# al-mcintyre/mCaller

Measured on NVIDIA B200. Metric: per-read site calls/sec, higher is better.
Workload: dtype f64

## Files before the change

### include/mcaller_b200.h

```cpp
#ifndef MCALLER_B200_H
#define MCALLER_B200_H

#include <stdint.h>

#ifdef __cplusplus
extern "C" {
#endif

#define MC_ABI_VERSION 3

#define MC_TILE_BYTES 3840
#define MC_TEXT_PAD 4096
#define MC_MAXK 8

enum {
    MC_OK = 0,
    MC_EINVAL = -1,
    MC_ECUDA = -2,
    MC_ECAPACITY = -3
};

typedef struct mc_refindex {
    int32_t n_contigs;
    int32_t k;
    const uint8_t *d_names;
    const int32_t *d_name_off;
    const int64_t *d_base;
    const int32_t *d_len;
    const uint32_t *d_site_fwd;
    const uint32_t *d_site_rev;
    const uint32_t *d_cand;
    const uint32_t *d_rank_fwd;
    const uint32_t *d_rank_rev;
    const uint8_t *d_bases;
    int64_t total_bits;
} mc_refindex;

typedef struct mc_record {
    uint32_t line_lo;
    uint16_t line_hi;
    uint16_t name_off;
    int32_t pos;
    int32_t event_idx;
    double diff;
    uint16_t name_len;
    uint16_t contig;
    uint8_t flags;
    uint8_t kbits_fwd;
    uint8_t kbits_rev;
    uint8_t pad;
} mc_record;

#define MC_RF_EQ 1u
#define MC_RF_CAND 2u
#define MC_RF_BADNUM 4u
#define MC_RF_BADIDX 8u
#define MC_RF_RAW 16u
#define MC_RF_NEWREAD 32u
#define MC_RF_SEGKNOWN 64u

enum {
    MC_C_LINES = 0,
    MC_C_KEPT,
    MC_C_RECORDS,
    MC_C_SHORT,
    MC_C_UNKNOWN_CONTIG,
    MC_C_NNN,
    MC_C_BADPOS,
    MC_C_LONGLINE,
    MC_C_OVERFLOW,
    MC_C_RUN_CURSOR,
    MC_C_QUIET,
    MC_C_COUNT = 16
};

typedef struct mc_call {
    int64_t read_off;
    double prob;
    double feat[MC_MAXK + 1];
    int32_t read_len;
    int32_t mpos;
    int32_t site;
    uint32_t close_rec;
    uint16_t win_contig;
    uint16_t chrom_contig;
    uint8_t kind;
    uint8_t rev;
    uint8_t n_empty;
    uint8_t empty_mask;
    uint8_t model_sel;
    uint8_t label;
    uint8_t err;
    uint8_t pad0;
    uint32_t seg;
    uint32_t pad1;
    uint32_t pad2;
} mc_call;

enum { MC_CALL = 0, MC_TOO_MANY_SKIPS = 1, MC_MULTI_M = 2, MC_NONE = 3  };
#define MC_CE_CONTEXT 1u
#define MC_CE_MODELKEY 2u
#define MC_CE_BADNUM 4u
#define MC_CE_COLUMN 8u
#define MC_CE_SPACING 16u

enum { MC_MLP = 0, MC_LR = 1, MC_GNB = 2, MC_RF = 3 };
enum { MC_ACT_IDENTITY = 0, MC_ACT_LOGISTIC = 1, MC_ACT_TANH = 2, MC_ACT_RELU = 3 };
typedef struct mc_model {
    int32_t kind;
    int32_t n_in;
    int32_t n_layers;
    int32_t hidden_act;
    int32_t sizes[8];
    const double *d_weights;
    const double *d_biases;
    int32_t n_trees;
    int32_t max_nodes;
    const int32_t *d_tree_off;
    const int32_t *d_left;
    const int32_t *d_right;
    const int32_t *d_feature;
    const double *d_threshold;
    const double *d_leaf_p1;
} mc_model;

typedef struct mc_qual_entry {
    uint64_t hash;
    uint32_t check;
    uint32_t len;
    double qual;
} mc_qual_entry;


int mc_version(void);
int mc_sizeof(int what);
const char *mc_last_error(void);

int mc_read_u64(const uint64_t *d_src, int64_t n, uint64_t *h_dst, void *stream);

int mc_scan(const uint8_t *d_text, int64_t nbytes, const mc_refindex *ref, int dense,
            mc_record *d_rec, int64_t rec_cap, uint32_t *d_tile_tab , uint32_t *d_run_tab ,
            uint64_t *d_counters, void *stream);

int mc_scan_run_len(int64_t nbytes);

int mc_scan_set_run_len(int run_len);

int64_t mc_num_tiles(int64_t nbytes);

int64_t mc_workspace_bytes(int64_t n);

int mc_order_records(const uint8_t *d_text, int64_t nbytes, const mc_refindex *ref, const uint32_t *d_tile_tab, int64_t n_tiles,
                     uint32_t *d_run_tab, int run_len, const mc_record *d_rec_in, int64_t rec_in_cap, const uint64_t *d_scan_counters,
                     mc_record *d_rec_out, int64_t rec_out_cap, uint64_t *d_n_out, uint32_t *d_seg_flags ,
                     uint32_t *d_run_first , void *d_ws, void *stream);

int mc_segment_reads(const uint8_t *d_text, mc_record *d_rec, const uint64_t *d_n_records, int64_t rec_cap,
                     uint32_t *d_seg_flags , const uint32_t *d_run_first, int64_t n_runs,
                     uint32_t *d_seg_start, uint64_t *d_nseg, void *d_ws, void *stream);

int mc_segment_quality(const uint8_t *d_text, const mc_record *d_rec, const uint32_t *d_seg_start, const uint64_t *d_nseg,
                       int64_t seg_cap, const mc_qual_entry *d_table, int64_t table_size, double *d_seg_qual, uint64_t *d_err,
                       void *stream);

int mc_build_windows(const mc_record *d_rec, const uint64_t *d_n_records, int64_t rec_cap, const uint32_t *d_seg_start,
                     const uint64_t *d_nseg, int64_t seg_cap, const double *d_seg_qual, const mc_refindex *ref, int skip_thresh,
                     double qual_thresh, int two_models, mc_call *d_calls, int64_t call_cap, uint32_t *d_seg_count,
                     uint64_t *d_ncalls, void *d_ws, double *d_spill, int64_t spill_cap, void *stream);

typedef struct mc_carry {
    mc_call row;
    uint32_t valid;
    int32_t first_kept_contig;
    uint64_t chunks;
    uint64_t pad[6];
} mc_carry;
int mc_carry_reset(mc_carry *d_carry, void *stream);
int mc_carry_rows(mc_call *d_rows, const uint64_t *d_ncalls, const mc_record *d_rec, const uint64_t *d_n_records,
                  const uint32_t *d_seg_start, const uint64_t *d_nseg, const double *d_seg_qual, double qual_thresh,
                  mc_carry *d_carry, uint64_t *d_nrows_out, const uint64_t *d_abort, void *stream);
int mc_chunk_guard(const uint64_t *d_counters, int64_t rec_cap, const uint64_t *d_n_records, int64_t rec_out_cap,
                   const uint64_t *d_nseg, int64_t seg_cap, const uint64_t *d_ncalls, int64_t call_cap, uint64_t *d_abort,
                   uint64_t *d_sticky , void *stream);
int mc_carry_close(mc_carry *d_carry, int closing_contig, const int64_t *d_next_contigs, int from, int count, mc_call *d_row_out,
                   uint32_t *d_depth, uint32_t *d_meth, uint64_t *d_first, int64_t n_sites, uint64_t *d_row_base, void *stream);

int64_t mc_classify_workspace_bytes(int64_t row_cap);
int mc_classify(mc_call *d_calls, const uint64_t *d_nrows, int64_t row_cap, const mc_model *models, void *d_ws, void *stream);

int mc_hist_accumulate(const mc_call *d_calls, const uint64_t *d_nrows, int64_t row_cap, uint32_t *d_depth, uint32_t *d_meth,
                       uint64_t *d_first, int64_t n_sites, uint64_t *d_row_base, mc_call *d_odd, int64_t odd_cap, uint64_t *d_n_odd,
                       const uint64_t *d_abort , void *stream);

int mc_bed_select(const uint32_t *d_depth, const uint32_t *d_meth, int64_t n_sites, int64_t depth_thresh, double mod_thresh,
                  int control, uint8_t *d_flags, uint64_t *d_count, void *stream);

int mc_count_calls(const mc_call *d_calls, const uint64_t *d_nrows, int64_t row_cap, uint64_t *d_out, void *stream);

typedef struct mc_locus_entry {
    unsigned long long hash;
    unsigned long long first_off;
    unsigned long long check;
    uint32_t depth;
    uint32_t meth;
} mc_locus_entry;

typedef struct mc_diffs_row {
    uint64_t line_off;
    uint32_t slot;
    uint32_t values_off;
    uint32_t values_len;
    uint32_t prob_off;
    uint32_t prob_len;
    uint32_t pad;
} mc_diffs_row;
int mc_diffs_aggregate_ex(const uint8_t *d_text, int64_t nbytes, int64_t base_off, const uint64_t *d_posset, int64_t posset_size,
                          mc_locus_entry *d_table, int64_t table_size, uint64_t *d_counters, void *stream);
int mc_diffs_rehash(const mc_locus_entry *d_old, int64_t old_size, mc_locus_entry *d_table, int64_t table_size,
                    uint64_t *d_counters, void *stream);
int mc_diffs_rows(const uint8_t *d_text, int64_t nbytes, const uint64_t *d_posset, int64_t posset_size,
                  const mc_locus_entry *d_table, int64_t table_size, mc_diffs_row *d_rows, int64_t row_cap, uint64_t *d_nrows,
                  void *stream);
int mc_diffs_colstats(const uint8_t *d_text, const mc_diffs_row *d_rows, const uint32_t *d_order, int64_t n_rows,
                      const uint32_t *d_locus_off, int64_t n_loci, int ncols, double *d_vals, uint32_t *d_ncol,
                      double *d_stats, uint64_t *d_counters, void *stream);

int64_t mc_format_rows(const mc_call *h_calls, int64_t n_calls, const uint8_t *h_text, const uint8_t *carry_name,
                       int32_t carry_name_len, const char *const *contig_names, const char *const *marked_fwd,
                       const char *const *marked_rev, const int64_t *contig_len, int32_t n_contigs, int32_t k,
                       const char *base_label, const char *mod_label, int32_t with_prob, int32_t max_threads, char *out,
                       int64_t out_cap);

int64_t mc_fastq_tiles(int64_t nbytes);
int mc_fastq_index(const uint8_t *d_text, int64_t nbytes, uint32_t *d_tile_cnt, uint32_t *d_tile_off, uint64_t *d_line_start,
                   int64_t line_cap, uint64_t *d_n_newlines, void *d_ws, void *stream);
int mc_fastq_quality(const uint8_t *d_text, int64_t nbytes, const uint64_t *d_line_start, int64_t n_lines, mc_qual_entry *d_table,
                     int64_t table_size, uint32_t *d_owner, double *d_rec_mean, uint64_t *d_stats, void *stream);

#define MC_TRAIN_HIDDEN 100
#define MC_TRAIN_BATCH 200
typedef struct mc_train_job {
    const double *d_x;
    const double *d_y;
    double *d_w;
    double *d_loss_curve;
    int64_t idx_off;
    int32_t n, d;
    int32_t max_iter, n_iter_no_change;
    double alpha, lr, tol;
    double best_loss;
    int32_t n_iter, no_improve, stopped, pad;
} mc_train_job;

int mc_mlp_train_init(mc_train_job *d_jobs, int32_t n_jobs, void *stream);
int mc_mlp_train_epochs(mc_train_job *d_jobs, int32_t n_jobs, const int32_t *d_idx, int32_t epochs, void *stream);

typedef struct mc_synth_spec {
    uint64_t seed;
    int32_t n_contigs;
    int32_t len_min, len_max, p_skip, p_nnn, margin;
    int32_t meth;
    const uint8_t *d_names;
    const int32_t *d_name_off;
    const int32_t *d_contig_len;
    const int64_t *d_read_bounds;
    const int64_t *d_gbase;
    const uint8_t *d_genome;
    const uint32_t *d_meth_fwd;
    const uint32_t *d_meth_rev;
    const int32_t *d_model_mean;
    const int32_t *d_model_sd;
} mc_synth_spec;

int mc_synth_genome(const mc_synth_spec *spec, uint8_t *d_genome_out, int64_t total_bits, void *stream);
int mc_synth_sizes(const mc_synth_spec *spec, int64_t read0, int64_t n, int64_t n_total_reads, uint64_t *d_sizes, void *stream);
int mc_synth_write(const mc_synth_spec *spec, int64_t read0, int64_t n, int64_t n_total_reads, const uint64_t *d_offsets,
                   uint8_t *d_text, void *stream);

#ifdef __cplusplus
}
#endif
#endif
```

### mcaller_b200/_lib.py

```python
import ctypes as C
import os

import numpy as np

HERE = os.path.dirname(os.path.abspath(__file__))
LIB_PATH = os.environ.get("MCALLER_B200_LIB") or os.path.join(HERE, "libmcaller_b200.so")

MC_TILE_BYTES = 3840
MC_TEXT_PAD = 4096
MC_MAXK = 8
MC_C_COUNT = 16
COUNTER_NAMES = ["lines", "kept", "records", "short", "unknown_contig", "nnn", "badpos", "longline", "overflow", "run_cursor", "quiet_chunks"]

MC_ABI_VERSION = 3
MC_CALL, MC_TOO_MANY_SKIPS, MC_MULTI_M, MC_NONE = 0, 1, 2, 3
MC_CE_CONTEXT, MC_CE_MODELKEY, MC_CE_BADNUM, MC_CE_COLUMN, MC_CE_SPACING = 1, 2, 4, 8, 16
MC_MLP, MC_LR, MC_GNB, MC_RF = 0, 1, 2, 3
PENDING = 0xFFFFFFFF


class RefIndex(C.Structure):
    _fields_ = [("n_contigs", C.c_int32), ("k", C.c_int32), ("d_names", C.c_void_p), ("d_name_off", C.c_void_p),
                ("d_base", C.c_void_p), ("d_len", C.c_void_p), ("d_site_fwd", C.c_void_p), ("d_site_rev", C.c_void_p),
                ("d_cand", C.c_void_p), ("d_rank_fwd", C.c_void_p), ("d_rank_rev", C.c_void_p), ("d_bases", C.c_void_p),
                ("total_bits", C.c_int64)]


class Model(C.Structure):
    _fields_ = [("kind", C.c_int32), ("n_in", C.c_int32), ("n_layers", C.c_int32), ("hidden_act", C.c_int32),
                ("sizes", C.c_int32 * 8), ("d_weights", C.c_void_p), ("d_biases", C.c_void_p), ("n_trees", C.c_int32),
                ("max_nodes", C.c_int32), ("d_tree_off", C.c_void_p), ("d_left", C.c_void_p), ("d_right", C.c_void_p),
                ("d_feature", C.c_void_p), ("d_threshold", C.c_void_p), ("d_leaf_p1", C.c_void_p)]


class SynthSpec(C.Structure):
    _fields_ = [("seed", C.c_uint64), ("n_contigs", C.c_int32), ("len_min", C.c_int32), ("len_max", C.c_int32),
                ("p_skip", C.c_int32), ("p_nnn", C.c_int32), ("margin", C.c_int32), ("meth", C.c_int32),
                ("d_names", C.c_void_p), ("d_name_off", C.c_void_p), ("d_contig_len", C.c_void_p),
                ("d_read_bounds", C.c_void_p), ("d_gbase", C.c_void_p), ("d_genome", C.c_void_p),
                ("d_meth_fwd", C.c_void_p), ("d_meth_rev", C.c_void_p), ("d_model_mean", C.c_void_p),
                ("d_model_sd", C.c_void_p)]


RECORD_DTYPE = np.dtype([("line_lo", "<u4"), ("line_hi", "<u2"), ("name_off", "<u2"), ("pos", "<i4"), ("event_idx", "<i4"),
                         ("diff", "<f8"), ("name_len", "<u2"), ("contig", "<u2"), ("flags", "u1"), ("kbits_fwd", "u1"), ("kbits_rev", "u1"), ("pad", "u1")])
assert RECORD_DTYPE.itemsize == 32

CALL_DTYPE = np.dtype([("read_off", "<i8"), ("prob", "<f8"), ("feat", "<f8", (MC_MAXK + 1,)), ("read_len", "<i4"),
                       ("mpos", "<i4"), ("site", "<i4"), ("close_rec", "<u4"), ("win_contig", "<u2"), ("chrom_contig", "<u2"),
                       ("kind", "u1"), ("rev", "u1"), ("n_empty", "u1"), ("empty_mask", "u1"), ("model_sel", "u1"),
                       ("label", "u1"), ("err", "u1"), ("pad0", "u1"), ("seg", "<u4"), ("pad1", "<u4"), ("pad2", "<u4")])
assert CALL_DTYPE.itemsize == 128

class LocusEntry(C.Structure):
    _fields_ = [("hash", C.c_uint64), ("first_off", C.c_uint64), ("check", C.c_uint64), ("depth", C.c_uint32), ("meth", C.c_uint32)]


class TrainJob(C.Structure):
    _fields_ = [("d_x", C.c_void_p), ("d_y", C.c_void_p), ("d_w", C.c_void_p), ("d_loss_curve", C.c_void_p), ("idx_off", C.c_int64),
                ("n", C.c_int32), ("d", C.c_int32), ("max_iter", C.c_int32), ("n_iter_no_change", C.c_int32), ("alpha", C.c_double),
                ("lr", C.c_double), ("tol", C.c_double), ("best_loss", C.c_double), ("n_iter", C.c_int32), ("no_improve", C.c_int32),
                ("stopped", C.c_int32), ("pad", C.c_int32)]


MC_TRAIN_HIDDEN, MC_TRAIN_BATCH = 100, 200

CARRY_BYTES = 192

QUAL_DTYPE = np.dtype([("hash", "<u8"), ("check", "<u4"), ("len", "<u4"), ("qual", "<f8")])
assert QUAL_DTYPE.itemsize == 24
DIFFS_ROW_DTYPE = np.dtype([("line_off", "<u8"), ("slot", "<u4"), ("values_off", "<u4"), ("values_len", "<u4"), ("prob_off", "<u4"),
                            ("prob_len", "<u4"), ("pad", "<u4")])
assert DIFFS_ROW_DTYPE.itemsize == 32


class McallerCudaError(RuntimeError):
    pass


_lib = None

_PROTOS = {
    "mc_version": (C.c_int, []),
    "mc_sizeof": (C.c_int, [C.c_int]),
    "mc_last_error": (C.c_char_p, []),
    "mc_read_u64": (C.c_int, [C.c_void_p, C.c_int64, C.c_void_p, C.c_void_p]),
    "mc_scan": (C.c_int, [C.c_void_p, C.c_int64, C.POINTER(RefIndex), C.c_int, C.c_void_p, C.c_int64, C.c_void_p, C.c_void_p, C.c_void_p,
                          C.c_void_p]),
    "mc_scan_run_len": (C.c_int, [C.c_int64]),
    "mc_scan_set_run_len": (C.c_int, [C.c_int]),
    "mc_num_tiles": (C.c_int64, [C.c_int64]),
    "mc_workspace_bytes": (C.c_int64, [C.c_int64]),
    "mc_order_records": (C.c_int, [C.c_void_p, C.c_int64, C.POINTER(RefIndex), C.c_void_p, C.c_int64, C.c_void_p, C.c_int, C.c_void_p,
                                   C.c_int64, C.c_void_p, C.c_void_p, C.c_int64, C.c_void_p, C.c_void_p, C.c_void_p, C.c_void_p, C.c_void_p]),
    "mc_segment_reads": (C.c_int, [C.c_void_p, C.c_void_p, C.c_void_p, C.c_int64, C.c_void_p, C.c_void_p, C.c_int64, C.c_void_p, C.c_void_p,
                                   C.c_void_p, C.c_void_p]),
    "mc_segment_quality": (C.c_int, [C.c_void_p, C.c_void_p, C.c_void_p, C.c_void_p, C.c_int64, C.c_void_p, C.c_int64, C.c_void_p,
                                     C.c_void_p, C.c_void_p]),
    "mc_build_windows": (C.c_int, [C.c_void_p, C.c_void_p, C.c_int64, C.c_void_p, C.c_void_p, C.c_int64, C.c_void_p, C.POINTER(RefIndex),
                                   C.c_int, C.c_double, C.c_int, C.c_void_p, C.c_int64, C.c_void_p, C.c_void_p, C.c_void_p, C.c_void_p,
                                   C.c_int64, C.c_void_p]),
    "mc_carry_reset": (C.c_int, [C.c_void_p, C.c_void_p]),
    "mc_carry_rows": (C.c_int, [C.c_void_p, C.c_void_p, C.c_void_p, C.c_void_p, C.c_void_p, C.c_void_p, C.c_void_p, C.c_double, C.c_void_p,
                                C.c_void_p, C.c_void_p, C.c_void_p]),
    "mc_chunk_guard": (C.c_int, [C.c_void_p, C.c_int64, C.c_void_p, C.c_int64, C.c_void_p, C.c_int64, C.c_void_p, C.c_int64, C.c_void_p,
                                 C.c_void_p, C.c_void_p]),
    "mc_carry_close": (C.c_int, [C.c_void_p, C.c_int, C.c_void_p, C.c_int, C.c_int, C.c_void_p, C.c_void_p, C.c_void_p, C.c_void_p,
                                 C.c_int64, C.c_void_p, C.c_void_p]),
    "mc_classify_workspace_bytes": (C.c_int64, [C.c_int64]),
    "mc_classify": (C.c_int, [C.c_void_p, C.c_void_p, C.c_int64, C.POINTER(Model), C.c_void_p, C.c_void_p]),
    "mc_hist_accumulate": (C.c_int, [C.c_void_p, C.c_void_p, C.c_int64, C.c_void_p, C.c_void_p, C.c_void_p, C.c_int64, C.c_void_p,
                                     C.c_void_p, C.c_int64, C.c_void_p, C.c_void_p, C.c_void_p]),
    "mc_count_calls": (C.c_int, [C.c_void_p, C.c_void_p, C.c_int64, C.c_void_p, C.c_void_p]),
    "mc_bed_select": (C.c_int, [C.c_void_p, C.c_void_p, C.c_int64, C.c_int64, C.c_double, C.c_int, C.c_void_p, C.c_void_p, C.c_void_p]),
    "mc_format_rows": (C.c_int64, [C.c_void_p, C.c_int64, C.c_void_p, C.c_void_p, C.c_int32, C.c_void_p, C.c_void_p, C.c_void_p, C.c_void_p,
                                   C.c_int32, C.c_int32, C.c_char_p, C.c_char_p, C.c_int32, C.c_int32, C.c_void_p, C.c_int64]),
    "mc_fastq_tiles": (C.c_int64, [C.c_int64]),
    "mc_fastq_index": (C.c_int, [C.c_void_p, C.c_int64, C.c_void_p, C.c_void_p, C.c_void_p, C.c_int64, C.c_void_p, C.c_void_p, C.c_void_p]),
    "mc_fastq_quality": (C.c_int, [C.c_void_p, C.c_int64, C.c_void_p, C.c_int64, C.c_void_p, C.c_int64, C.c_void_p, C.c_void_p, C.c_void_p,
                                   C.c_void_p]),
    "mc_synth_genome": (C.c_int, [C.POINTER(SynthSpec), C.c_void_p, C.c_int64, C.c_void_p]),
    "mc_synth_sizes": (C.c_int, [C.POINTER(SynthSpec), C.c_int64, C.c_int64, C.c_int64, C.c_void_p, C.c_void_p]),
    "mc_synth_write": (C.c_int, [C.POINTER(SynthSpec), C.c_int64, C.c_int64, C.c_int64, C.c_void_p, C.c_void_p, C.c_void_p]),
    "mc_diffs_aggregate_ex": (C.c_int, [C.c_void_p, C.c_int64, C.c_int64, C.c_void_p, C.c_int64, C.c_void_p, C.c_int64, C.c_void_p, C.c_void_p]),
    "mc_diffs_rehash": (C.c_int, [C.c_void_p, C.c_int64, C.c_void_p, C.c_int64, C.c_void_p, C.c_void_p]),
    "mc_diffs_rows": (C.c_int, [C.c_void_p, C.c_int64, C.c_void_p, C.c_int64, C.c_void_p, C.c_int64, C.c_void_p, C.c_int64, C.c_void_p,
                                C.c_void_p]),
    "mc_mlp_train_init": (C.c_int, [C.c_void_p, C.c_int32, C.c_void_p]),
    "mc_mlp_train_epochs": (C.c_int, [C.c_void_p, C.c_int32, C.c_void_p, C.c_int32, C.c_void_p]),
    "mc_diffs_colstats": (C.c_int, [C.c_void_p, C.c_void_p, C.c_void_p, C.c_int64, C.c_void_p, C.c_int64, C.c_int, C.c_void_p, C.c_void_p,
                                    C.c_void_p, C.c_void_p, C.c_void_p]),
}

EXPORTS = sorted(_PROTOS)


def load(path=LIB_PATH):
    if not os.path.exists(path):
        raise McallerCudaError("libmcaller_b200.so is not built (%s); run `python -m mcaller_b200.build` -- there is no CPU fallback" % path)
    lib = C.CDLL(path)
    for name, (res, args) in _PROTOS.items():
        fn = getattr(lib, name)
        fn.restype = res
        fn.argtypes = args
    return lib


def lib():
    global _lib
    if _lib is None:
        _lib = load()
        if _lib.mc_version() != MC_ABI_VERSION:
            raise McallerCudaError("ABI version mismatch")
    return _lib


def check(rc):
    if rc != 0:
        raise McallerCudaError("libmcaller_b200: rc=%d %s" % (rc, lib().mc_last_error().decode(errors="replace")))
```

### mcaller_b200/csrc/classify.cu

```cuda
#include "common.cuh"

namespace {

constexpr int MAX_WIDTH = 512;
constexpr int WARPS = 8;

__device__ __forceinline__ double activate(double v, int act) {
    switch (act) {
        case MC_ACT_TANH: return mc_tanh(v);
        case MC_ACT_LOGISTIC: return mc_expit(v);
        case MC_ACT_RELU: return v > 0.0 ? v : 0.0;
        default: return v;
    }
}

template <bool STAGED>
__global__ void __launch_bounds__(WARPS * 32)
k_mlp(mc_call *__restrict__ calls, int64_t n_cap, const unsigned long long *__restrict__ d_n, mc_model m0, mc_model m1, int width, int nw0,
      int nb0, int nw1, int nb1, int alias) {
    extern __shared__ __align__(16) double s_mlp[];
    const int64_t n = mc_dev_count(d_n, n_cap);
    const int warp = threadIdx.x >> 5, lane = threadIdx.x & 31;
    double *s_act = s_mlp;
    if (STAGED) {
        for (int j = threadIdx.x; j < nw0; j += WARPS * 32) s_mlp[j] = __ldg(m0.d_weights + j);
        for (int j = threadIdx.x; j < nb0; j += WARPS * 32) s_mlp[nw0 + j] = __ldg(m0.d_biases + j);
        for (int j = threadIdx.x; j < nw1; j += WARPS * 32) s_mlp[nw0 + nb0 + j] = __ldg(m1.d_weights + j);
        for (int j = threadIdx.x; j < nb1; j += WARPS * 32) s_mlp[nw0 + nb0 + nw1 + j] = __ldg(m1.d_biases + j);
        s_act = s_mlp + nw0 + nb0 + nw1 + nb1;
        __syncthreads();
    }
    double *a = s_act + (size_t)warp * 2 * width, *b = a + width;
    const int64_t stride = (int64_t)gridDim.x * WARPS;
    int64_t i = (int64_t)blockIdx.x * WARPS + warp;
    auto fetch = [&](int64_t idx, double &f, int &kind_sel) {
        f = 0.0;
        kind_sel = -1;
        if (idx < n) {
            const mc_call &c = calls[idx];
            kind_sel = c.kind == MC_CALL ? (int)c.model_sel : -1;
            if (lane <= MC_MAXK) f = c.feat[lane];
        }
    };
    double f_cur;
    int ks_cur;
    fetch(i, f_cur, ks_cur);
    for (; i < n; i += stride) {
        double f_next;
        int ks_next;
        fetch(i + stride, f_next, ks_next);
        if (ks_cur >= 0) {
            const mc_model &m = ks_cur ? m1 : m0;
            const double *w = STAGED ? ((ks_cur && !alias) ? s_mlp + nw0 + nb0 : s_mlp) : m.d_weights;
            const double *bi = STAGED ? ((ks_cur && !alias) ? s_mlp + nw0 + nb0 + nw1 : s_mlp + nw0) : m.d_biases;
            auto ld = [&](const double *p) { return STAGED ? *p : __ldg(p); };
            double *x = a, *y = b;
            if (lane < m.sizes[0]) x[lane] = f_cur;
            __syncwarp();
            for (int l = 0; l < m.n_layers; ++l) {
                const int ni = m.sizes[l], no = m.sizes[l + 1];
                const bool last = (l + 1 == m.n_layers);
                if (no >= 8) {
                    for (int o0 = 0; o0 < no; o0 += 128) {
                        double acc[4];
#pragma unroll
                        for (int j = 0; j < 4; ++j) acc[j] = 0.0;
                        for (int k = 0; k < ni; ++k) {
                            const double ak = x[k];
#pragma unroll
                            for (int j = 0; j < 4; ++j) {
                                const int o = o0 + lane + 32 * j;
                                if (o < no) acc[j] = fma(ak, ld(w + (size_t)k * no + o), acc[j]);
                            }
                        }
#pragma unroll
                        for (int j = 0; j < 4; ++j) {
                            const int o = o0 + lane + 32 * j;
                            if (o < no) {
                                const double z = acc[j] + ld(bi + o);
                                y[o] = last ? z : activate(z, m.hidden_act);
                            }
                        }
                    }
                } else {
                    for (int o = 0; o < no; ++o) {
                        double acc = 0.0;
                        for (int k = lane; k < ni; k += 32) acc = fma(x[k], ld(w + (size_t)k * no + o), acc);
                        for (int d = 16; d > 0; d >>= 1) acc += __shfl_xor_sync(0xffffffffu, acc, d);
                        acc += ld(bi + o);
                        if (lane == 0) y[o] = last ? acc : activate(acc, m.hidden_act);
                    }
                }
                __syncwarp();
                double *t = x; x = y; y = t;
                w += (size_t)ni * no;
                bi += no;
            }
            const double out = mc_expit(x[0]);
            __syncwarp();
            if (lane == 0) {
                mc_call &c = calls[i];
                c.prob = out;
                c.label = (uint8_t)(out >= 0.5);
            }
        }
        f_cur = f_next;
        ks_cur = ks_next;
    }
}

constexpr int MLP_MAX_IN = MC_MAXK + 1;

__global__ void __launch_bounds__(256) k_call_index(const mc_call *__restrict__ calls, int64_t n_cap, const unsigned long long *__restrict__ d_n,
                                                   uint32_t *__restrict__ idx, unsigned long long *__restrict__ d_nidx) {
    __shared__ unsigned int s_warp[8];
    __shared__ unsigned long long s_base;
    const int64_t n = mc_dev_count(d_n, n_cap);
    if ((int64_t)blockIdx.x * blockDim.x >= n) return;
    const int64_t i = (int64_t)blockIdx.x * blockDim.x + threadIdx.x;
    const bool is_call = i < n && calls[i].kind == MC_CALL;
    const int lane = threadIdx.x & 31, wid = threadIdx.x >> 5;
    const uint32_t m = __ballot_sync(0xffffffffu, is_call);
    if (lane == 0) s_warp[wid] = __popc(m);
    __syncthreads();
    if (threadIdx.x == 0) {
        unsigned int tot = 0u;
        for (int w = 0; w < 8; ++w) { const unsigned int c = s_warp[w]; s_warp[w] = tot; tot += c; }
        s_base = tot ? atomicAdd(d_nidx, (unsigned long long)tot) : 0ull;
    }
    __syncthreads();
    if (is_call) idx[s_base + s_warp[wid] + __popc(m & ((1u << lane) - 1u))] = (uint32_t)i;
}
__global__ void __launch_bounds__(WARPS * 32)
k_mlp_1hidden(mc_call *__restrict__ calls, const uint32_t *__restrict__ idx, const unsigned long long *__restrict__ d_nidx, mc_model m0,
              mc_model m1, int nw0, int nb0, int nw1, int nb1, int alias) {
    extern __shared__ __align__(16) double s_mlp[];
    const int64_t n = (int64_t)*d_nidx;
    if ((int64_t)blockIdx.x * WARPS * 8 >= n) return;
    for (int j = threadIdx.x; j < nw0; j += WARPS * 32) s_mlp[j] = __ldg(m0.d_weights + j);
    for (int j = threadIdx.x; j < nb0; j += WARPS * 32) s_mlp[nw0 + j] = __ldg(m0.d_biases + j);
    for (int j = threadIdx.x; j < nw1; j += WARPS * 32) s_mlp[nw0 + nb0 + j] = __ldg(m1.d_weights + j);
    for (int j = threadIdx.x; j < nb1; j += WARPS * 32) s_mlp[nw0 + nb0 + nw1 + j] = __ldg(m1.d_biases + j);
    __syncthreads();
    const int warp = threadIdx.x >> 5, lane = threadIdx.x & 31, g = lane & 3, grp = lane >> 2;
    const int64_t stride = (int64_t)gridDim.x * WARPS * 8;
    for (int64_t base = ((int64_t)blockIdx.x * WARPS + warp) * 8; base < n; base += stride) {
        int64_t i = base + grp;
        int ks = -1;
        double x[MLP_MAX_IN];
#pragma unroll
        for (int k = 0; k < MLP_MAX_IN; ++k) x[k] = 0.0;
        if (i < n) {
            i = (int64_t)__ldg(idx + i);
            const mc_call &c = calls[i];
            ks = (int)c.model_sel;
#pragma unroll
            for (int k = 0; k < MLP_MAX_IN; ++k) x[k] = c.feat[k];
        }
        const bool second = ks > 0;
        const mc_model &m = second ? m1 : m0;
        const int ni = m.sizes[0], H = m.sizes[1], act = m.hidden_act;
        const double *w0 = (second && !alias) ? s_mlp + nw0 + nb0 : s_mlp;
        const double *b0 = (second && !alias) ? s_mlp + nw0 + nb0 + nw1 : s_mlp + nw0;
        const double *w1 = w0 + (size_t)ni * H, *b1 = b0 + H;
        double out = 0.0;
        if (ks >= 0) {
            for (int o0 = g; o0 < H; o0 += 16) {
                double z[4];
#pragma unroll
                for (int j = 0; j < 4; ++j) z[j] = 0.0;
#pragma unroll
                for (int k = 0; k < MLP_MAX_IN; ++k) {
                    if (k < ni) {
#pragma unroll
                        for (int j = 0; j < 4; ++j) {
                            const int o = o0 + 4 * j;
                            if (o < H) z[j] = fma(x[k], w0[(size_t)k * H + o], z[j]);
                        }
                    }
                }
#pragma unroll
                for (int j = 0; j < 4; ++j) {
                    const int o = o0 + 4 * j;
                    if (o < H) out = fma(act == MC_ACT_TANH ? mc_tanh(z[j] + b0[o]) : activate(z[j] + b0[o], act), w1[o], out);
                }
            }
        }
        out += __shfl_xor_sync(0xffffffffu, out, 1);
        out += __shfl_xor_sync(0xffffffffu, out, 2);
        if (ks >= 0 && g == 0) {
            const double p = mc_expit(out + b1[0]);
            mc_call &c = calls[i];
            c.prob = p;
            c.label = (uint8_t)(p >= 0.5);
        }
    }
}

__global__ void __launch_bounds__(256) k_linear(mc_call *__restrict__ calls, int64_t n_cap, const unsigned long long *__restrict__ d_n,
                                               mc_model m0, mc_model m1) {
    const int64_t n = mc_dev_count(d_n, n_cap);
    const int64_t i = (int64_t)blockIdx.x * blockDim.x + threadIdx.x;
    if (i >= n) return;
    mc_call &c = calls[i];
    if (c.kind != MC_CALL) return;
    const mc_model &m = c.model_sel ? m1 : m0;
    double p;
    if (m.kind == MC_LR) {
        double z = __ldg(m.d_biases);
        for (int k = 0; k < m.n_in; ++k) z += c.feat[k] * __ldg(m.d_weights + k);
        p = mc_expit(z);
    } else {
        const double *theta = m.d_weights, *var = m.d_weights + 2 * m.n_in;
        double jll[2];
        for (int cl = 0; cl < 2; ++cl) {
            double nij = 0.0, s = 0.0;
            for (int k = 0; k < m.n_in; ++k) nij += log(2.0 * 3.14159265358979323846 * __ldg(var + cl * m.n_in + k));
            nij *= -0.5;
            for (int k = 0; k < m.n_in; ++k) {
                const double d = c.feat[k] - __ldg(theta + cl * m.n_in + k);
                s += d * d / __ldg(var + cl * m.n_in + k);
            }
            jll[cl] = __ldg(m.d_biases + cl) + nij - 0.5 * s;
        }
        const double mx = jll[0] > jll[1] ? jll[0] : jll[1];
        const double lse = mx + log(exp(jll[0] - mx) + exp(jll[1] - mx));
        p = exp(jll[1] - lse);
    }
    c.prob = p;
    c.label = (uint8_t)(p >= 0.5);
}

__global__ void __launch_bounds__(256)
k_rf(mc_call *__restrict__ calls, int64_t n_cap, const unsigned long long *__restrict__ d_n, mc_model m0, mc_model m1, int max_nodes) {
    extern __shared__ __align__(16) uint8_t rf_smem[];
    const int64_t n = mc_dev_count(d_n, n_cap);
    if ((int64_t)blockIdx.x * blockDim.x >= n) return;
    double *s_thr = reinterpret_cast<double *>(rf_smem);
    double *s_p1 = s_thr + max_nodes;
    int32_t *s_left = reinterpret_cast<int32_t *>(s_p1 + max_nodes);
    int32_t *s_right = s_left + max_nodes;
    int32_t *s_feat = s_right + max_nodes;
    const int64_t i = (int64_t)blockIdx.x * blockDim.x + threadIdx.x;
    const bool active = i < n && calls[i].kind == MC_CALL;
    float x[MC_MAXK + 1];
    int sel = 0;
    if (active) {
        sel = calls[i].model_sel;
        for (int k = 0; k <= MC_MAXK; ++k) x[k] = (float)calls[i].feat[k];
    }
    double acc = 0.0;
    for (int pass = 0; pass < 2; ++pass) {
        const mc_model &m = pass ? m1 : m0;
        const int any = __syncthreads_or(active && sel == pass);
        if (!any || m.n_trees == 0) continue;
        for (int t = 0; t < m.n_trees; ++t) {
            const int o0 = __ldg(m.d_tree_off + t), nn = __ldg(m.d_tree_off + t + 1) - o0;
            __syncthreads();
            for (int j = threadIdx.x; j < nn; j += blockDim.x) {
                s_thr[j] = __ldg(m.d_threshold + o0 + j);
                s_p1[j] = __ldg(m.d_leaf_p1 + o0 + j);
                s_left[j] = __ldg(m.d_left + o0 + j);
                s_right[j] = __ldg(m.d_right + o0 + j);
                s_feat[j] = __ldg(m.d_feature + o0 + j);
            }
            __syncthreads();
            if (active && sel == pass) {
                int node = 0;
                while (s_left[node] >= 0) node = ((double)x[s_feat[node]] <= s_thr[node]) ? s_left[node] : s_right[node];
                acc += s_p1[node];
            }
        }
    }
    if (active) {
        const mc_model &m = sel ? m1 : m0;
        const double p = acc / (double)m.n_trees;
        calls[i].prob = p;
        calls[i].label = (uint8_t)(p >= 0.5);
    }
}

__global__ void __launch_bounds__(256)
k_hist(const mc_call *__restrict__ calls, int64_t n_cap, const unsigned long long *__restrict__ d_n, uint32_t *__restrict__ depth,
       uint32_t *__restrict__ meth, unsigned long long *__restrict__ first, int64_t n_sites, const unsigned long long *__restrict__ d_row_base,
       mc_call *__restrict__ d_odd, unsigned long long odd_cap, unsigned long long *__restrict__ d_n_odd,
       const unsigned long long *__restrict__ d_abort) {
    if (d_abort && *d_abort) return;
    const int64_t n = mc_dev_count(d_n, n_cap);
    const int64_t i = (int64_t)blockIdx.x * blockDim.x + threadIdx.x;
    if (i >= n) return;
    const mc_call &c = calls[i];
    if (c.kind != MC_CALL || c.close_rec == 0xFFFFFFFFu || c.err) return;
    const unsigned long long row = *d_row_base + (unsigned long long)i;
    if (c.chrom_contig != c.win_contig || c.site < 0 || c.site >= n_sites) {
        const unsigned long long slot = atomicAdd(d_n_odd, 1ull);
        if (slot < odd_cap) {
            mc_call o = c;
            o.pad1 = (uint32_t)(row & 0xFFFFFFFFull);
            o.pad2 = (uint32_t)(row >> 32);
            d_odd[slot] = o;
        }
        return;
    }
    atomicAdd(depth + c.site, 1u);
    if (c.label) atomicAdd(meth + c.site, 1u);
    atomicMin(first + c.site, row);
}
__global__ void k_advance_base(unsigned long long *d_row_base, const unsigned long long *d_n, const unsigned long long *d_abort) {
    if (d_abort && *d_abort) return;
    *d_row_base += *d_n;
}
__global__ void k_chunk_guard(const unsigned long long *__restrict__ counters, unsigned long long rec_cap,
                              const unsigned long long *__restrict__ d_n_records, unsigned long long rec_out_cap,
                              const unsigned long long *__restrict__ d_nseg, unsigned long long seg_cap,
                              const unsigned long long *__restrict__ d_ncalls, unsigned long long call_cap,
                              unsigned long long *__restrict__ d_abort, unsigned long long *__restrict__ d_sticky) {
    const bool bad = counters[MC_C_OVERFLOW] != 0ull || counters[MC_C_RECORDS] > rec_cap || *d_n_records > rec_out_cap ||
                     *d_nseg > seg_cap || d_ncalls[0] > call_cap || d_ncalls[1] != 0ull;
    *d_abort = bad ? 1ull : 0ull;
    if (bad && d_sticky) *d_sticky = 1ull;
}

__global__ void __launch_bounds__(256) k_count_calls(const mc_call *__restrict__ calls, int64_t n_cap, const unsigned long long *__restrict__ d_n,
                                                    unsigned long long *__restrict__ out) {
    __shared__ unsigned int s[7];
    const int64_t n = mc_dev_count(d_n, n_cap);
    if ((int64_t)blockIdx.x * blockDim.x >= n) return;
    if (threadIdx.x < 7) s[threadIdx.x] = 0u;
    __syncthreads();
    const int64_t i = (int64_t)blockIdx.x * blockDim.x + threadIdx.x;
    if (i < n) {
        const mc_call &c = calls[i];
        if (c.kind == MC_CALL) {
            atomicAdd(&s[c.close_rec == 0xFFFFFFFFu ? 1 : 0], 1u);
            if (c.label && c.close_rec != 0xFFFFFFFFu) atomicAdd(&s[5], 1u);
        } else if (c.kind == MC_TOO_MANY_SKIPS) atomicAdd(&s[c.close_rec == 0xFFFFFFFFu ? 6 : 2], 1u);
        else if (c.kind == MC_MULTI_M) atomicAdd(&s[3], 1u);
        if (c.kind != MC_NONE && c.err) atomicAdd(&s[4], 1u);
    }
    __syncthreads();
    if (threadIdx.x < 7 && s[threadIdx.x]) atomicAdd(out + threadIdx.x, (unsigned long long)s[threadIdx.x]);
}

__global__ void __launch_bounds__(256)
k_bed_select(const uint32_t *__restrict__ depth, const uint32_t *__restrict__ meth, int64_t n_sites, long long depth_thresh,
             double mod_thresh, int control, uint8_t *__restrict__ flags, unsigned long long *__restrict__ d_count) {
    const int64_t i = (int64_t)blockIdx.x * blockDim.x + threadIdx.x;
    bool keep = false;
    if (i < n_sites) {
        const uint32_t d = depth[i];
        if (d > 0u && (long long)d >= depth_thresh) {
            const double frac = __ddiv_rn((double)meth[i], (double)d);
            keep = control ? (frac < mod_thresh) : (frac >= mod_thresh);
        }
        flags[i] = keep ? 1 : 0;
    }
    const unsigned m = __ballot_sync(0xffffffffu, keep);
    if ((threadIdx.x & 31) == 0 && m) atomicAdd(d_count, (unsigned long long)__popc(m));
}

__device__ __forceinline__ void copy_row(mc_call *dst, const mc_call *src) {
    const uint4 *s4 = reinterpret_cast<const uint4 *>(src);
    uint4 *d4 = reinterpret_cast<uint4 *>(dst);
#pragma unroll
    for (int j = 0; j < 8; ++j) d4[j] = s4[j];
}

__global__ void __launch_bounds__(32)
k_carry_rows(mc_call *__restrict__ rows, const unsigned long long *__restrict__ d_ncalls, const mc_record *__restrict__ rec,
             const unsigned long long *__restrict__ d_n_records, const uint32_t *__restrict__ seg_start,
             const unsigned long long *__restrict__ d_nseg, const double *__restrict__ seg_qual, double qual_thresh,
             mc_carry *__restrict__ carry, unsigned long long *__restrict__ d_nrows_out, const unsigned long long *__restrict__ d_abort) {
    const int lane = threadIdx.x;
    if (d_abort && *d_abort) {
        if (lane == 0) *d_nrows_out = 0ull;
        return;
    }
    const unsigned long long n_rows = *d_ncalls, n_rec = *d_n_records, n_seg = *d_nseg;
    long long fk_rec = -1;
    if (n_rec > 0 && n_seg > 0) {
        if (!(qual_thresh > 0.0)) fk_rec = 0;
        else {
            for (unsigned long long s0 = 0; s0 < n_seg && fk_rec < 0; s0 += 32) {
                const unsigned long long sg = s0 + lane;
                const bool ok = sg < n_seg && !(seg_qual[sg] < qual_thresh);
                const uint32_t m = __ballot_sync(0xffffffffu, ok);
                if (m) fk_rec = (long long)seg_start[s0 + (__ffs(m) - 1)];
            }
        }
    }
    if (lane != 0) return;
    int fk_contig = -1;
    if (fk_rec >= 0) fk_contig = (int)rec[fk_rec].contig;
    mc_call *slot0 = rows;
    bool resolved = false;
    if (carry->valid && fk_contig >= 0) {
        copy_row(slot0, &carry->row);
        slot0->chrom_contig = (uint16_t)fk_contig;
        slot0->close_rec = (uint32_t)fk_rec;
        slot0->read_off = -1;
        slot0->seg = 0xFFFFFFFFu;
        carry->valid = 0u;
        resolved = true;
    }
    if (!resolved) {
        mc_call z;
        memset(&z, 0, sizeof(z));
        z.kind = MC_NONE;
        z.site = -1;
        copy_row(slot0, &z);
    }
    if (n_rows > 0) {
        const mc_call *last = rows + n_rows;
        if (last->close_rec == 0xFFFFFFFFu && (last->kind == MC_CALL || last->kind == MC_TOO_MANY_SKIPS)) {
            copy_row(&carry->row, last);
            carry->valid = 1u;
        }
    }
    if (carry->first_kept_contig < 0 && fk_contig >= 0) carry->first_kept_contig = fk_contig;
    carry->chunks += 1ull;
    *d_nrows_out = n_rows + 1ull;
}

__global__ void k_carry_reset(mc_carry *carry) {
    memset(carry, 0, sizeof(*carry));
    carry->first_kept_contig = -1;
    carry->row.kind = MC_NONE;
}

__global__ void k_carry_close(mc_carry *__restrict__ carry, int closing_contig, const long long *__restrict__ d_next, int from, int count,
                              mc_call *__restrict__ out, uint32_t *__restrict__ depth, uint32_t *__restrict__ meth,
                              unsigned long long *__restrict__ first, int64_t n_sites, unsigned long long *__restrict__ d_row_base) {
    const unsigned long long row_index = d_row_base ? *d_row_base : 0ull;
    int cc = closing_contig;
    if (cc < 0 && d_next) {
        for (int j = from; j < count; ++j) {
            if (d_next[j] >= 0) { cc = (int)d_next[j]; break; }
        }
    }
    mc_call z;
    memset(&z, 0, sizeof(z));
    z.kind = MC_NONE;
    z.site = -1;
    if (!carry->valid || cc < 0) {
        copy_row(out, &z);
        carry->valid = 0u;
        return;
    }
    copy_row(out, &carry->row);
    out->chrom_contig = (uint16_t)cc;
    out->close_rec = 0u;
    out->read_off = -1;
    out->seg = 0xFFFFFFFFu;
    out->pad1 = (uint32_t)(row_index & 0xFFFFFFFFull);
    out->pad2 = (uint32_t)(row_index >> 32);
    carry->valid = 0u;
    if (out->kind == MC_CALL && !out->err && depth && out->chrom_contig == out->win_contig && out->site >= 0 && out->site < n_sites) {
        atomicAdd(depth + out->site, 1u);
        if (out->label) atomicAdd(meth + out->site, 1u);
        atomicMin(first + out->site, row_index);
    }
    if (d_row_base) *d_row_base = row_index + 1ull;
}

}

extern "C" int mc_count_calls(const mc_call *d_calls, const uint64_t *d_nrows, int64_t row_cap, uint64_t *d_out, void *stream) {
    MC_REQUIRE(d_calls && d_nrows && d_out, "null pointer");
    if (row_cap <= 0) return MC_OK;
    k_count_calls<<<(unsigned)((row_cap + 255) / 256), 256, 0, (cudaStream_t)stream>>>(
        d_calls, row_cap, reinterpret_cast<const unsigned long long *>(d_nrows), reinterpret_cast<unsigned long long *>(d_out));
    MC_LAUNCH_CHECK();
    return MC_OK;
}

extern "C" int mc_carry_reset(mc_carry *d_carry, void *stream) {
    MC_REQUIRE(d_carry, "null pointer");
    k_carry_reset<<<1, 1, 0, (cudaStream_t)stream>>>(d_carry);
    MC_LAUNCH_CHECK();
    return MC_OK;
}

extern "C" int mc_carry_rows(mc_call *d_rows, const uint64_t *d_ncalls, const mc_record *d_rec, const uint64_t *d_n_records,
                             const uint32_t *d_seg_start, const uint64_t *d_nseg, const double *d_seg_qual, double qual_thresh,
                             mc_carry *d_carry, uint64_t *d_nrows_out, const uint64_t *d_abort, void *stream) {
    MC_REQUIRE(d_rows && d_ncalls && d_rec && d_n_records && d_seg_start && d_nseg && d_seg_qual && d_carry && d_nrows_out, "null pointer");
    k_carry_rows<<<1, 32, 0, (cudaStream_t)stream>>>(d_rows, reinterpret_cast<const unsigned long long *>(d_ncalls), d_rec,
                                                     reinterpret_cast<const unsigned long long *>(d_n_records), d_seg_start,
                                                     reinterpret_cast<const unsigned long long *>(d_nseg), d_seg_qual, qual_thresh, d_carry,
                                                     reinterpret_cast<unsigned long long *>(d_nrows_out),
                                                     reinterpret_cast<const unsigned long long *>(d_abort));
    MC_LAUNCH_CHECK();
    return MC_OK;
}

extern "C" int mc_bed_select(const uint32_t *d_depth, const uint32_t *d_meth, int64_t n_sites, int64_t depth_thresh, double mod_thresh,
                             int control, uint8_t *d_flags, uint64_t *d_count, void *stream) {
    MC_REQUIRE(d_depth && d_meth && d_flags && d_count, "null pointer");
    MC_CUDA_CHECK(cudaMemsetAsync(d_count, 0, 8, (cudaStream_t)stream));
    if (n_sites <= 0) return MC_OK;
    k_bed_select<<<(unsigned)((n_sites + 255) / 256), 256, 0, (cudaStream_t)stream>>>(d_depth, d_meth, n_sites, (long long)depth_thresh, mod_thresh,
                                                                                      control, d_flags, reinterpret_cast<unsigned long long *>(d_count));
    MC_LAUNCH_CHECK();
    return MC_OK;
}

extern "C" int mc_chunk_guard(const uint64_t *d_counters, int64_t rec_cap, const uint64_t *d_n_records, int64_t rec_out_cap,
                              const uint64_t *d_nseg, int64_t seg_cap, const uint64_t *d_ncalls, int64_t call_cap, uint64_t *d_abort,
                              uint64_t *d_sticky, void *stream) {
    MC_REQUIRE(d_counters && d_n_records && d_nseg && d_ncalls && d_abort, "null pointer");
    k_chunk_guard<<<1, 1, 0, (cudaStream_t)stream>>>(reinterpret_cast<const unsigned long long *>(d_counters), (unsigned long long)rec_cap,
                                                    reinterpret_cast<const unsigned long long *>(d_n_records), (unsigned long long)rec_out_cap,
                                                    reinterpret_cast<const unsigned long long *>(d_nseg), (unsigned long long)seg_cap,
                                                    reinterpret_cast<const unsigned long long *>(d_ncalls), (unsigned long long)call_cap,
                                                    reinterpret_cast<unsigned long long *>(d_abort), reinterpret_cast<unsigned long long *>(d_sticky));
    MC_LAUNCH_CHECK();
    return MC_OK;
}

extern "C" int mc_carry_close(mc_carry *d_carry, int closing_contig, const int64_t *d_next_contigs, int from, int count,
                              mc_call *d_row_out, uint32_t *d_depth, uint32_t *d_meth, uint64_t *d_first, int64_t n_sites,
                              uint64_t *d_row_base, void *stream) {
    MC_REQUIRE(d_carry && d_row_out, "null pointer");
    MC_REQUIRE(!d_depth || (d_meth && d_first), "histogram needs depth, meth and first");
    k_carry_close<<<1, 1, 0, (cudaStream_t)stream>>>(d_carry, closing_contig, reinterpret_cast<const long long *>(d_next_contigs), from, count,
                                                    d_row_out, d_depth, d_meth, reinterpret_cast<unsigned long long *>(d_first), n_sites,
                                                    reinterpret_cast<unsigned long long *>(d_row_base));
    MC_LAUNCH_CHECK();
    return MC_OK;
}

extern "C" int64_t mc_classify_workspace_bytes(int64_t row_cap) { return 256 + 4 * (row_cap < 1 ? 1 : row_cap); }

extern "C" int mc_classify(mc_call *d_calls, const uint64_t *d_nrows, int64_t n_calls , const mc_model *models,
                           void *d_ws, void *stream) {
    MC_REQUIRE(d_calls && d_nrows && models && d_ws, "null pointer");
    if (n_calls <= 0) return MC_OK;
    cudaStream_t st = (cudaStream_t)stream;
    const unsigned long long *dn = reinterpret_cast<const unsigned long long *>(d_nrows);
    const mc_model &m0 = models[0], &m1 = models[1];
    MC_REQUIRE(m0.kind == m1.kind, "models 0 ('MH') and 1 ('MG') are of different kinds");
    MC_REQUIRE(m0.n_in >= 1 && m0.n_in <= MC_MAXK + 1, "model 0 ('MH') input width out of range");
    MC_REQUIRE(m1.n_in == m0.n_in, "models 0 ('MH') and 1 ('MG') take different input widths");
    switch (m0.kind) {
        case MC_MLP: {
            for (const mc_model *m : {&m0, &m1}) {
                MC_REQUIRE(m->n_layers >= 1 && m->n_layers < 8, "MLP depth out of range");
                MC_REQUIRE(m->sizes[0] == m->n_in, "MLP input layer does not match its input width");
                for (int l = 0; l <= m->n_layers; ++l) MC_REQUIRE(m->sizes[l] >= 1 && m->sizes[l] <= MAX_WIDTH, "MLP layer too wide");
                MC_REQUIRE(m->sizes[m->n_layers] == 1, "MLP must have one logistic output");
            }
            int width = 8;
            for (int l = 0; l <= m0.n_layers; ++l) width = m0.sizes[l] > width ? m0.sizes[l] : width;
            for (int l = 0; l <= m1.n_layers; ++l) width = m1.sizes[l] > width ? m1.sizes[l] : width;
            width = (width + 3) & ~3;
            auto count = [](const mc_model &m, int &nw, int &nb) {
                nw = nb = 0;
                if (m.kind != MC_MLP) return;
                for (int l = 0; l < m.n_layers; ++l) { nw += m.sizes[l] * m.sizes[l + 1]; nb += m.sizes[l + 1]; }
            };
            int nw0, nb0, nw1, nb1;
            count(m0, nw0, nb0);
            count(m1, nw1, nb1);
            const int alias = (m1.kind == MC_MLP && m1.d_weights == m0.d_weights) ? 1 : 0;
            if (alias) nw1 = nb1 = 0;
            int dev = 0, sms = 0;
            MC_CUDA_CHECK(cudaGetDevice(&dev));
            MC_CUDA_CHECK(cudaDeviceGetAttribute(&sms, cudaDevAttrMultiProcessorCount, dev));
            const size_t act_bytes = sizeof(double) * 2 * (size_t)width * WARPS;
            const size_t staged_bytes = act_bytes + sizeof(double) * (size_t)(nw0 + nb0 + nw1 + nb1);
            int64_t blocks = (n_calls + WARPS - 1) / WARPS;
            if (blocks > (int64_t)sms * 8) blocks = (int64_t)sms * 8;
            auto one_hidden = [](const mc_model &m) {
                return m.kind == MC_MLP && m.n_layers == 2 && m.sizes[0] <= MLP_MAX_IN && m.sizes[2] == 1;
            };
            const size_t weight_bytes = sizeof(double) * (size_t)(nw0 + nb0 + nw1 + nb1);
            if (one_hidden(m0) && (alias || one_hidden(m1)) && weight_bytes <= 100 * 1024) {
                int64_t b2 = (n_calls + WARPS * 8 - 1) / (WARPS * 8);
                if (b2 > (int64_t)sms * 8) b2 = (int64_t)sms * 8;
                unsigned long long *d_nidx = reinterpret_cast<unsigned long long *>(d_ws);
                uint32_t *d_idx = reinterpret_cast<uint32_t *>(reinterpret_cast<uint8_t *>(d_ws) + 256);
                MC_CUDA_CHECK(cudaMemsetAsync(d_nidx, 0, 8, st));
                k_call_index<<<(unsigned)((n_calls + 255) / 256), 256, 0, st>>>(d_calls, n_calls, dn, d_idx, d_nidx);
                MC_LAUNCH_CHECK();
                MC_CUDA_CHECK(cudaFuncSetAttribute(k_mlp_1hidden, cudaFuncAttributeMaxDynamicSharedMemorySize, (int)weight_bytes));
                k_mlp_1hidden<<<(unsigned)b2, WARPS * 32, weight_bytes, st>>>(d_calls, d_idx, d_nidx, m0, m1, nw0, nb0, nw1, nb1, alias);
            } else if (staged_bytes <= 100 * 1024) {
                MC_CUDA_CHECK(cudaFuncSetAttribute(k_mlp<true>, cudaFuncAttributeMaxDynamicSharedMemorySize, (int)staged_bytes));
                k_mlp<true><<<(unsigned)blocks, WARPS * 32, staged_bytes, st>>>(d_calls, n_calls, dn, m0, m1, width, nw0, nb0, nw1, nb1, alias);
            } else {
                k_mlp<false><<<(unsigned)blocks, WARPS * 32, act_bytes, st>>>(d_calls, n_calls, dn, m0, m1, width, 0, 0, 0, 0, 0);
            }
            break;
        }
        case MC_LR:
        case MC_GNB:
            k_linear<<<(unsigned)((n_calls + 255) / 256), 256, 0, st>>>(d_calls, n_calls, dn, m0, m1);
            break;
        case MC_RF: {
            int mx = m0.max_nodes > m1.max_nodes ? m0.max_nodes : m1.max_nodes;
            MC_REQUIRE(mx >= 1, "RF max_nodes missing");
            const size_t smem = (size_t)mx * (8 + 8 + 4 + 4 + 4);
            MC_REQUIRE(smem <= 200 * 1024, "RF tree too large for shared-memory staging");
            MC_CUDA_CHECK(cudaFuncSetAttribute(k_rf, cudaFuncAttributeMaxDynamicSharedMemorySize, (int)smem));
            k_rf<<<(unsigned)((n_calls + 255) / 256), 256, smem, st>>>(d_calls, n_calls, dn, m0, m1, mx);
            break;
        }
        default:
            MC_REQUIRE(false, "unknown model kind");
    }
    MC_LAUNCH_CHECK();
    return MC_OK;
}

extern "C" int mc_hist_accumulate(const mc_call *d_calls, const uint64_t *d_nrows, int64_t row_cap, uint32_t *d_depth, uint32_t *d_meth,
                                  uint64_t *d_first, int64_t n_sites, uint64_t *d_row_base, mc_call *d_odd, int64_t odd_cap,
                                  uint64_t *d_n_odd, const uint64_t *d_abort, void *stream) {
    MC_REQUIRE(d_calls && d_nrows && d_depth && d_meth && d_first && d_row_base && d_odd && d_n_odd, "null pointer");
    if (row_cap <= 0) return MC_OK;
    k_hist<<<(unsigned)((row_cap + 255) / 256), 256, 0, (cudaStream_t)stream>>>(
        d_calls, row_cap, reinterpret_cast<const unsigned long long *>(d_nrows), d_depth, d_meth,
        reinterpret_cast<unsigned long long *>(d_first), n_sites, reinterpret_cast<const unsigned long long *>(d_row_base), d_odd,
        (unsigned long long)odd_cap, reinterpret_cast<unsigned long long *>(d_n_odd), reinterpret_cast<const unsigned long long *>(d_abort));
    MC_LAUNCH_CHECK();
    k_advance_base<<<1, 1, 0, (cudaStream_t)stream>>>(reinterpret_cast<unsigned long long *>(d_row_base),
                                                      reinterpret_cast<const unsigned long long *>(d_nrows),
                                                      reinterpret_cast<const unsigned long long *>(d_abort));
    MC_LAUNCH_CHECK();
    return MC_OK;
}
```

### mcaller_b200/csrc/common.cuh

```cuda
#pragma once
#include <cuda_runtime.h>
#include <stdint.h>
#include <stdio.h>
#include "../../include/mcaller_b200.h"

void mc_set_error(const char *fmt, ...);

#define MC_CUDA_CHECK(expr)                                                                  \
    do {                                                                                     \
        cudaError_t _e = (expr);                                                             \
        if (_e != cudaSuccess) {                                                             \
            mc_set_error("%s:%d %s -> %s", __FILE__, __LINE__, #expr, cudaGetErrorString(_e)); \
            return MC_ECUDA;                                                                 \
        }                                                                                    \
    } while (0)

#define MC_LAUNCH_CHECK() MC_CUDA_CHECK(cudaGetLastError())

#define MC_REQUIRE(cond, msg)                       \
    do {                                            \
        if (!(cond)) {                              \
            mc_set_error("%s: %s", __func__, msg);  \
            return MC_EINVAL;                       \
        }                                           \
    } while (0)

__device__ __forceinline__ uint32_t mc_kmer_bits(const uint32_t *__restrict__ bm, int64_t g, int k) {
    int64_t w = g >> 5;
    int b = (int)(g & 31);
    uint32_t lo = __ldg(bm + w), hi = __ldg(bm + w + 1);
    uint32_t v = __funnelshift_r(lo, hi, b);
    return v & ((1u << k) - 1u);
}

template <int THREADS>
__device__ __forceinline__ int mc_block_exscan(int v, int *s_warp , int &total) {
    const int lane = threadIdx.x & 31, wid = threadIdx.x >> 5;
    int inc = v;
#pragma unroll
    for (int d = 1; d < 32; d <<= 1) {
        int t = __shfl_up_sync(0xffffffffu, inc, d);
        if (lane >= d) inc += t;
    }
    if (lane == 31) s_warp[wid] = inc;
    __syncthreads();
    if (wid == 0) {
        int x = (lane < THREADS / 32) ? s_warp[lane] : 0;
        int xi = x;
#pragma unroll
        for (int d = 1; d < 32; d <<= 1) {
            int t = __shfl_up_sync(0xffffffffu, xi, d);
            if (lane >= d) xi += t;
        }
        if (lane < THREADS / 32) s_warp[lane] = xi - x;
        if (lane == 31) s_warp[THREADS / 32] = xi;
    }
    __syncthreads();
    total = s_warp[THREADS / 32];
    int res = s_warp[wid] + inc - v;
    __syncthreads();
    return res;
}

int mc_exscan_u32(const uint32_t *d_in, uint32_t *d_out, int64_t n_cap, const uint64_t *d_n ,
                  uint64_t *d_total , void *d_ws, cudaStream_t st);
int64_t mc_exscan_ws_bytes(int64_t n);

__device__ __forceinline__ int64_t mc_dev_count(const unsigned long long *d_n, int64_t cap) {
    const unsigned long long v = *d_n;
    return v < (unsigned long long)cap ? (int64_t)v : cap;
}

__device__ __forceinline__ int64_t mc_rec_line(const mc_record &r) { return ((int64_t)r.line_hi << 32) | (int64_t)r.line_lo; }

struct mc_read_key {
    unsigned long long hash;
    uint32_t check;
    uint32_t len;
};
__device__ __forceinline__ mc_read_key mc_read_key_of(const uint8_t *p, int64_t max_len) {
    unsigned long long h = 14695981039346656037ull, h2 = 0x84222325cbf29ce4ull;
    int64_t len = 0;
    for (; len < max_len; ++len) {
        const unsigned c = __ldg(p + len);
        if (c <= 0x20u || c == ':' || c == '_') break;
        h = (h ^ c) * 1099511628211ull;
        h2 = (h2 ^ c) * 1099511628211ull;
    }
    return {h == 0ull ? 1ull : h, (uint32_t)(h2 >> 32), (uint32_t)len};
}

template <class F>
__device__ __forceinline__ double mc_pairwise_block(F f, int64_t i0, int64_t n) {
    if (n < 8) {
        double res = 0.0;
        for (int64_t i = 0; i < n; ++i) res = __dadd_rn(res, f(i0 + i));
        return res;
    }
    double r[8];
#pragma unroll
    for (int j = 0; j < 8; ++j) r[j] = f(i0 + j);
    int64_t i = 8;
    for (; i < n - (n % 8); i += 8) {
#pragma unroll
        for (int j = 0; j < 8; ++j) r[j] = __dadd_rn(r[j], f(i0 + i + j));
    }
    double res = __dadd_rn(__dadd_rn(__dadd_rn(r[0], r[1]), __dadd_rn(r[2], r[3])), __dadd_rn(__dadd_rn(r[4], r[5]), __dadd_rn(r[6], r[7])));
    for (; i < n; ++i) res = __dadd_rn(res, f(i0 + i));
    return res;
}
template <class F>
__device__ double mc_pairwise_sum(F f, int64_t i0, int64_t n) {
    if (n <= 128) return mc_pairwise_block(f, i0, n);
    constexpr int DEPTH = 40;
    int64_t st_i0[DEPTH], st_n[DEPTH];
    double st_left[DEPTH];
    int st_phase[DEPTH];
    int sp = 0;
    st_i0[0] = i0; st_n[0] = n; st_phase[0] = 0; st_left[0] = 0.0;
    double ret = 0.0;
    for (;;) {
        if (st_phase[sp] == 0) {
            if (st_n[sp] <= 128 || sp + 1 >= DEPTH) {
                ret = mc_pairwise_block(f, st_i0[sp], st_n[sp]);
            } else {
                int64_t n2 = st_n[sp] / 2;
                n2 -= n2 % 8;
                st_phase[sp] = 1;
                st_i0[sp + 1] = st_i0[sp]; st_n[sp + 1] = n2; st_phase[sp + 1] = 0;
                ++sp;
                continue;
            }
        }
        for (;;) {
            if (sp == 0) return ret;
            --sp;
            if (st_phase[sp] == 1) {
                int64_t n2 = st_n[sp] / 2;
                n2 -= n2 % 8;
                st_left[sp] = ret;
                st_phase[sp] = 2;
                st_i0[sp + 1] = st_i0[sp] + n2; st_n[sp + 1] = st_n[sp] - n2; st_phase[sp + 1] = 0;
                ++sp;
                break;
            }
            ret = __dadd_rn(st_left[sp], ret);
        }
    }
}

__device__ __forceinline__ double mc_expit(double x) { return x < 0.0 ? exp(x) / (1.0 + exp(x)) : 1.0 / (1.0 + exp(-x)); }

__device__ __forceinline__ double mc_tanh(double x) {
    double y = -2.0 * fabs(x);
    y = fmax(y, -80.0);
    const double n = rint(y * 1.4426950408889634074);
    double r = fma(n, -6.93147180369123816490e-01, y);
    r = fma(n, -1.90821492927058770002e-10, r);
    double p = 1.6059043836821613e-10;
    p = fma(p, r, 2.0876756987868100e-09);
    p = fma(p, r, 2.5052108385441720e-08);
    p = fma(p, r, 2.7557319223985890e-07);
    p = fma(p, r, 2.7557319223985893e-06);
    p = fma(p, r, 2.4801587301587302e-05);
    p = fma(p, r, 1.9841269841269841e-04);
    p = fma(p, r, 1.3888888888888889e-03);
    p = fma(p, r, 8.3333333333333332e-03);
    p = fma(p, r, 4.1666666666666664e-02);
    p = fma(p, r, 1.6666666666666666e-01);
    p = fma(p, r, 0.5);
    p = fma(p, r, 1.0);
    p = fma(p, r, 1.0);
    const double t = p * __longlong_as_double((long long)(1023 + (int)n) << 52);
    const double d = 1.0 + t, u = 1.0 - t;
    double rc = (double)__frcp_rn((float)d);
    double e = fma(-d, rc, 1.0);
    rc = fma(rc, e, rc);
    e = fma(-d, rc, 1.0);
    rc = fma(rc, e, rc);
    double q = u * rc;
    q = fma(fma(-d, q, u), rc, q);
    return copysign(q, x);
}
```

### mcaller_b200/csrc/windows.cu

```cuda
#include "common.cuh"

namespace {

#ifndef MC_WIN_ITEMS
#define MC_WIN_ITEMS 12
#endif
#ifndef MC_WIN_THREADS
#define MC_WIN_THREADS 128
#endif
#ifndef MC_WIN_BLOCKS
#define MC_WIN_BLOCKS 4
#endif
constexpr int WIN_THREADS = MC_WIN_THREADS, WIN_ITEMS = MC_WIN_ITEMS, WIN_RECS = WIN_THREADS * WIN_ITEMS;
constexpr int WIN_UNITS = WIN_RECS / 2 + 2;
static_assert(WIN_RECS < 65536, "unit / read counts of a block are packed in 16 bits");
constexpr uint32_t TAG_NONE = 0xFu;

__device__ __forceinline__ uint4 stage_word(const mc_record *p) {
    const uint4 a = __ldg(reinterpret_cast<const uint4 *>(p)), b = __ldg(reinterpret_cast<const uint4 *>(p) + 1);
    return make_uint4(a.z, a.w, (b.w & 0x00FFFFFFu) | (TAG_NONE << 24), b.z >> 16);
}
__device__ __forceinline__ double stage_diff(const mc_record *p) {
    const uint4 b = __ldg(reinterpret_cast<const uint4 *>(p) + 1);
    return __longlong_as_double((long long)(((unsigned long long)b.y << 32) | b.x));
}

struct Counts {
    unsigned long long lo, hi;
};
__device__ __forceinline__ int cnt_get(const Counts &q, int c) { return (int)(((c < 4 ? q.lo : q.hi) >> (16 * (c & 3))) & 0xFFFFull); }
__device__ __forceinline__ void cnt_inc(Counts &q, int c) {
    if (cnt_get(q, c) < 65535) {
        const unsigned long long one = 1ull << (16 * (c & 3));
        if (c < 4) q.lo += one; else q.hi += one;
    }
}
__device__ __forceinline__ void cnt_clear(Counts &q, int c) {
    const unsigned long long m = ~(0xFFFFull << (16 * (c & 3)));
    if (c < 4) q.lo &= m; else q.hi &= m;
}
__device__ __forceinline__ int map_get(uint32_t mp, int c) { return (int)((mp >> (4 * c)) & 0xFu); }

__device__ __forceinline__ mc_record load_rec(const mc_record *p) {
    mc_record r;
    const uint4 *s = reinterpret_cast<const uint4 *>(p);
    uint4 a = __ldg(s), b = __ldg(s + 1);
    uint4 *d = reinterpret_cast<uint4 *>(&r);
    d[0] = a;
    d[1] = b;
    return r;
}

__device__ __forceinline__ uint8_t comp_base(uint8_t c) {
    switch (c) {
        case 'A': return 'T';
        case 'C': return 'G';
        case 'G': return 'C';
        case 'T': return 'A';
        case 'N': return 'N';
        default: return 0;
    }
}

__global__ void __launch_bounds__(128) k_first_m(const mc_record *__restrict__ rec, const uint32_t *__restrict__ seg_start, int64_t seg_cap,
                                                const unsigned long long *__restrict__ d_nseg, uint32_t *__restrict__ first_idx,
                                                int32_t *__restrict__ first_ind) {
    const int64_t n_seg = mc_dev_count(d_nseg, seg_cap);
    const int64_t seg = (int64_t)blockIdx.x * blockDim.x + threadIdx.x;
    if (seg >= n_seg) return;
    const uint32_t b = seg_start[seg], e = seg_start[seg + 1];
    uint32_t fi = 0xFFFFFFFFu;
    int32_t ev = 0;
    for (uint32_t i = b; i < e; ++i) {
        const uint4 c = __ldg(reinterpret_cast<const uint4 *>(rec + i) + 1);
        const uint32_t fl = c.w & 0xFFu;
        if (!(fl & MC_RF_CAND)) continue;
        const int rev = !(fl & MC_RF_EQ);
        const uint32_t bits = rev ? ((c.w >> 16) & 0xFFu) : ((c.w >> 8) & 0xFFu);
        if (bits) { fi = i; ev = (int32_t)__ldg(reinterpret_cast<const uint4 *>(rec + i)).w; break; }
    }
    first_idx[seg] = fi;
    first_ind[seg] = ev;
}

struct Spill {
    double *buf;
    unsigned long long cap;
    unsigned long long *cursor;
};

struct ColSrc {
    const uint4 *s_rec;
    const double *s_diff;
    const mc_record *rec;
    const uint8_t *g_tag;
    int64_t base;
};
__device__ __forceinline__ uint32_t cs_tag(const ColSrc &S, uint32_t i) {
    const int64_t j = (int64_t)i - S.base;
    return (j >= 0 && j < WIN_RECS) ? (S.s_rec[j].z >> 24) : (uint32_t)S.g_tag[i];
}
__device__ __forceinline__ double cs_diff(const ColSrc &S, uint32_t i) {
    const int64_t j = (int64_t)i - S.base;
    return (j >= 0 && j < WIN_RECS) ? S.s_diff[j] : stage_diff(S.rec + i);
}
__device__ __noinline__ double col_sum_big(const ColSrc S, uint32_t src, uint32_t unit_b, uint32_t upto, int n, Spill spill, uint32_t *err) {
    uint32_t f0 = upto;
    for (int need = n; need > 0 && f0 > unit_b;) {
        --f0;
        if (cs_tag(S, f0) == src) --need;
    }
    if (n >= 65535) { *err |= MC_CE_COLUMN; return 0.0; }
    double res = 0.0;
    if (n <= 128) {
        double r[8];
#pragma unroll
        for (int q = 0; q < 8; ++q) r[q] = 0.0;
        const int full = n - (n % 8);
        int t = 0;
        uint32_t j = f0;
        for (; j < upto && t < full; ++j) {
            if (cs_tag(S, j) != src) continue;
            const double v = cs_diff(S, j);
#pragma unroll
            for (int q = 0; q < 8; ++q)
                if ((t & 7) == q) r[q] = t < 8 ? v : __dadd_rn(r[q], v);
            ++t;
        }
        res = __dadd_rn(__dadd_rn(__dadd_rn(r[0], r[1]), __dadd_rn(r[2], r[3])), __dadd_rn(__dadd_rn(r[4], r[5]), __dadd_rn(r[6], r[7])));
        for (; j < upto; ++j)
            if (cs_tag(S, j) == src) res = __dadd_rn(res, cs_diff(S, j));
        return res;
    }
    const unsigned long long at = atomicAdd(spill.cursor, (unsigned long long)n);
    if (at + (unsigned long long)n > spill.cap) { *err |= MC_CE_COLUMN; return 0.0; }
    double *a = spill.buf + at;
    int t = 0;
    for (uint32_t j = f0; j < upto; ++j)
        if (cs_tag(S, j) == src) a[t++] = cs_diff(S, j);
    return mc_pairwise_sum([a](int64_t q) { return a[q]; }, 0, n);
}

template <bool WRITE>
__global__ void __launch_bounds__(WIN_THREADS, MC_WIN_BLOCKS)
k_windows(const mc_record *__restrict__ rec, int64_t rec_cap, const unsigned long long *__restrict__ d_n_records,
          const uint32_t *__restrict__ seg_start, int64_t seg_cap, const unsigned long long *__restrict__ d_nseg,
          const double *__restrict__ seg_qual, const uint32_t *__restrict__ first_idx, const int32_t *__restrict__ first_ind_arr,
          mc_refindex R, int skip_thresh, double qual_thresh, int two_models, mc_call *__restrict__ calls,
          unsigned long long call_cap, uint32_t *__restrict__ unit_cnt ,
          uint32_t *__restrict__ blk_tot, const uint32_t *__restrict__ blk_off, uint8_t *__restrict__ g_tag , Spill spill) {
    __shared__ uint32_t s_unit[WIN_UNITS];
    __shared__ uint32_t s_off[WIN_UNITS];
    __shared__ uint16_t s_seg[WIN_UNITS];
    __shared__ int s_warp[WIN_THREADS / 32 + 1];
    __shared__ int64_t s_seg0;
    extern __shared__ __align__(16) uint4 s_dyn[];
    uint4 *s_rec = s_dyn;
    double *s_diff = reinterpret_cast<double *>(s_dyn + WIN_RECS);
    double *s_seq = s_diff + WIN_RECS + threadIdx.x;
    const int k = R.k;
    const int64_t n_records = mc_dev_count(d_n_records, rec_cap), n_seg = mc_dev_count(d_nseg, seg_cap);
    const int64_t base = (int64_t)blockIdx.x * WIN_RECS;
    if (base >= n_records || n_seg <= 0) {
        if (!WRITE && threadIdx.x == 0) blk_tot[blockIdx.x] = 0u;
        return;
    }
    for (int j = threadIdx.x; j < WIN_RECS; j += WIN_THREADS) {
        const int64_t i = base + j;
        if (i < n_records) {
            s_rec[j] = stage_word(rec + i);
            if (WRITE) s_diff[j] = stage_diff(rec + i);
        } else {
            s_rec[j] = make_uint4(0u, 0u, TAG_NONE << 24, 0u);
        }
    }
    if (threadIdx.x == 0) {
        int64_t lo = 0, hi = n_seg - 1;
        while (lo < hi) {
            const int64_t mid = (lo + hi + 1) >> 1;
            if ((int64_t)__ldg(seg_start + mid) <= base) lo = mid; else hi = mid - 1;
        }
        s_seg0 = lo;
    }
    __syncthreads();
    auto rec_word = [&](uint32_t i) -> uint4 {
        const int64_t j = (int64_t)i - base;
        return (j >= 0 && j < WIN_RECS) ? s_rec[j] : stage_word(rec + i);
    };
    auto rec_diff = [&](uint32_t i) -> double {
        const int64_t j = (int64_t)i - base;
        return (WRITE && j >= 0 && j < WIN_RECS) ? s_diff[j] : stage_diff(rec + i);
    };
    auto tag_set = [&](uint32_t i, uint32_t t) {
        const int64_t j = (int64_t)i - base;
        if (j >= 0 && j < WIN_RECS) s_rec[j].z = (s_rec[j].z & 0x00FFFFFFu) | (t << 24);
        else g_tag[i] = (uint8_t)t;
    };
    auto tag_get = [&](uint32_t i) -> uint32_t {
        const int64_t j = (int64_t)i - base;
        return (j >= 0 && j < WIN_RECS) ? (s_rec[j].z >> 24) : (uint32_t)g_tag[i];
    };
    int nu;
    {
        const int j0 = threadIdx.x * WIN_ITEMS;
        const int64_t i0 = base + j0;
        uint32_t prev_cand = 0u;
        if (i0 > 0 && i0 <= n_records)
            prev_cand = (j0 > 0 ? s_rec[j0 - 1].z : __ldg(reinterpret_cast<const uint4 *>(rec + i0 - 1) + 1).w) & MC_RF_CAND;
        uint32_t umask = 0u, nmask = 0u;
#pragma unroll
        for (int j = 0; j < WIN_ITEMS; ++j) {
            const int64_t i = i0 + j;
            if (i < n_records) {
                const uint4 w = s_rec[j0 + j];
                const uint32_t fl = w.z & 0xFFu;
                const uint32_t cand = fl & MC_RF_CAND;
                bool u;
                if (i == 0 || (fl & MC_RF_NEWREAD)) {
                    if (i != base) nmask |= 1u << j;
                    u = cand != 0u;
                    if (!u) u = (int)w.x < k;
                } else {
                    u = cand != 0u && prev_cand == 0u;
                }
                if (u) umask |= 1u << j;
                prev_cand = cand;
            }
        }
        int total;
        const int off = mc_block_exscan<WIN_THREADS>(__popc(umask) | (__popc(nmask) << 16), s_warp, total);
        int ou = off & 0xFFFF;
        const int on = off >> 16;
        for (uint32_t m = umask; m; m &= m - 1u) {
            const int j = __ffs(m) - 1;
            if (ou < WIN_UNITS) {
                s_unit[ou] = (uint32_t)(i0 + j);
                s_seg[ou] = (uint16_t)(on + __popc(nmask & ((2u << j) - 1u)));
            }
            ++ou;
        }
        nu = total & 0xFFFF;
        if (nu > WIN_UNITS) nu = WIN_UNITS;
        __syncthreads();
    }
    if (WRITE) {
        constexpr int UPT = (WIN_UNITS + WIN_THREADS - 1) / WIN_THREADS;
        uint32_t v[UPT];
        int sum = 0;
#pragma unroll
        for (int j = 0; j < UPT; ++j) {
            const int u = threadIdx.x * UPT + j;
            v[j] = u < nu ? unit_cnt[s_unit[u]] : 0u;
            sum += (int)v[j];
        }
        int total;
        uint32_t run = blk_off[blockIdx.x] + (uint32_t)mc_block_exscan<WIN_THREADS>(sum, s_warp, total);
#pragma unroll
        for (int j = 0; j < UPT; ++j) {
            const int u = threadIdx.x * UPT + j;
            if (u < WIN_UNITS) s_off[u] = run;
            run += v[j];
        }
        __syncthreads();
    }
    int my_rows = 0;
    for (int un = threadIdx.x; un < nu; un += WIN_THREADS) {
    const uint32_t b = s_unit[un];
    const int64_t seg = s_seg0 + s_seg[un];
    const uint32_t seg_b = __ldg(seg_start + seg), e_read = __ldg(seg_start + seg + 1);
    const bool whole = (int)rec_word(seg_b).x < k;
    uint32_t n_out = 0;
    const double myq = seg_qual[seg];
    if (myq < qual_thresh || (whole && b != seg_b)) {
        if (!WRITE) unit_cnt[b] = 0u;
        continue;
    }
    uint32_t e = e_read;
    uint32_t out_pos = WRITE ? s_off[un] : 0u;
    const uint32_t fidx = __ldg(first_idx + seg);

    Counts cnts{0ull, 0ull};
    uint32_t mp = 0x76543210u;
    bool started = b > fidx;
    bool has_mpos = false;
    int mpos = 0, first_ind = started ? __ldg(first_ind_arr + seg) : 0, last_rev = 0, last_cid = 0;
    uint32_t name_rec = b;
    uint32_t sticky_err = 0u;

#define MPOS_TRUTHY (has_mpos && mpos != 0)

    auto col_mean = [&](int src, uint32_t upto, uint32_t &err) -> double {
        const int n = cnt_get(cnts, src);
        double res;
        if (n < 8) res = s_seq[src * WIN_THREADS];
        else {
            const ColSrc S{s_rec, s_diff, rec, g_tag, base};
            res = col_sum_big(S, (uint32_t)src, b, upto, n, spill, &err);
        }
        return __ddiv_rn(res, (double)n);
    };

    auto emit_window = [&](uint32_t close_idx, int chrom_cid, uint32_t upto) {
        int n_empty = 0;
        for (int c = 0; c < k; ++c) n_empty += (cnt_get(cnts, map_get(mp, c)) == 0);
        if (WRITE) {
            if (out_pos < call_cap) {
                mc_call &o = calls[out_pos];
                const mc_record nr = load_rec(rec + name_rec);
                o.read_off = mc_rec_line(nr) + nr.name_off;
                o.read_len = nr.name_len;
                o.prob = 0.0;
                o.mpos = mpos;
                o.close_rec = close_idx;
                o.win_contig = (uint16_t)last_cid;
                o.chrom_contig = (uint16_t)(chrom_cid < 0 ? 0xFFFF : chrom_cid);
                o.rev = (uint8_t)last_rev;
                o.n_empty = (uint8_t)n_empty;
                o.label = 0;
                o.pad0 = 0;
                o.seg = (uint32_t)seg;
                o.pad1 = 0;
                o.pad2 = 0;
                uint32_t err = sticky_err;
                uint32_t empty_mask = 0u;
                const int64_t g = __ldg(R.d_base + last_cid) + mpos;
                {
                    const uint32_t *bm = last_rev ? R.d_site_rev : R.d_site_fwd;
                    const uint32_t *rk = last_rev ? R.d_rank_rev : R.d_rank_fwd;
                    const uint32_t wbits = __ldg(bm + (g >> 5));
                    o.site = (int32_t)(__ldg(rk + (g >> 5)) + __popc(wbits & ((1u << (g & 31)) - 1u)));
                }
                if (n_empty <= skip_thresh) {
                    o.kind = MC_CALL;
                    for (int c = 0; c < k; ++c) {
                        const int src = map_get(mp, last_rev ? c : (k - 1 - c));
                        if (cnt_get(cnts, src) == 0) { o.feat[c] = 0.0; empty_mask |= 1u << c; }
                        else o.feat[c] = col_mean(src, upto, err);
                    }
                    o.feat[k] = myq;
                    for (int c = k + 1; c <= MC_MAXK; ++c) o.feat[c] = 0.0;
                    const int clen = __ldg(R.d_len + last_cid);
                    uint8_t nextb = 0;
                    if (mpos - k + 1 < 0 || mpos + k > clen) err |= MC_CE_CONTEXT;
                    else if (k < 2) {
                    } else if (!last_rev) {
                        const int64_t gn = g + 1;
                        nextb = ((__ldg(R.d_site_fwd + (gn >> 5)) >> (gn & 31)) & 1u) ? 'M' : __ldg(R.d_bases + gn);
                    } else {
                        const int64_t gn = g - 1;
                        nextb = ((__ldg(R.d_site_rev + (gn >> 5)) >> (gn & 31)) & 1u) ? 'M' : comp_base(__ldg(R.d_bases + gn));
                    }
                    if (!(err & MC_CE_CONTEXT) &&
                        !(nextb == 'A' || nextb == 'C' || nextb == 'G' || nextb == 'T' || nextb == 'M'))
                        err |= MC_CE_MODELKEY;
                    o.model_sel = (uint8_t)((two_models && nextb == 'G') ? 1 : 0);
                } else {
                    o.kind = MC_TOO_MANY_SKIPS;
                    for (int c = 0; c <= MC_MAXK; ++c) o.feat[c] = 0.0;
                    o.model_sel = 0;
                }
                o.empty_mask = (uint8_t)empty_mask;
                o.err = (uint8_t)err;
            }
            ++out_pos;
        }
        ++n_out;
    };
    auto emit_multi = [&]() {
        if (WRITE) {
            if (out_pos < call_cap) {
                mc_call &o = calls[out_pos];
                const mc_record nr = load_rec(rec + name_rec);
                o.read_off = mc_rec_line(nr) + nr.name_off;
                o.read_len = nr.name_len;
                o.prob = 0.0;
                for (int c = 0; c <= MC_MAXK; ++c) o.feat[c] = 0.0;
                o.mpos = mpos;
                o.site = -1;
                o.close_rec = 0u;
                o.win_contig = (uint16_t)last_cid;
                o.chrom_contig = (uint16_t)last_cid;
                o.kind = MC_MULTI_M;
                o.rev = (uint8_t)last_rev;
                o.n_empty = 0; o.empty_mask = 0; o.model_sel = 0; o.label = 0; o.err = 0; o.pad0 = 0;
                o.seg = (uint32_t)seg;
                o.pad1 = 0;
                o.pad2 = 0;
            }
            ++out_pos;
        }
        ++n_out;
    };
    auto reset_cols = [&]() { cnts.lo = 0ull; cnts.hi = 0ull; };

    auto tag_init = [&](uint32_t q) {
        if (WRITE && (int64_t)q - base >= WIN_RECS) g_tag[q] = (uint8_t)TAG_NONE;
    };
    uint32_t i = b;
    uint4 r = (b < e) ? rec_word(b) : make_uint4(0u, 0u, 0u, 0u);
    if (b < e) tag_init(b);
    auto advance = [&]() {
        ++i;
        if (i < e) { r = rec_word(i); tag_init(i); }
    };
    int rev = 0, first_m = -1, cid = 0, pos = 0;
    bool pending_close = false, handoff_done = false;
    auto feed = [&]() {
        if (first_m >= 0) {
            if (MPOS_TRUTHY && rev != last_rev) has_mpos = false;
            if (!MPOS_TRUTHY) { has_mpos = true; mpos = pos + first_m; }
            started = true;
            last_rev = rev;
            last_cid = cid;
            name_rec = i;
            if (r.z & MC_RF_BADNUM) sticky_err |= MC_CE_BADNUM;
            const int slot = map_get(mp, first_m);
            if (WRITE) {
                const double v = rec_diff(i);
                double *q = s_seq + slot * WIN_THREADS;
                *q = __dadd_rn(cnt_get(cnts, slot) == 0 ? 0.0 : *q, v);
                tag_set(i, (uint32_t)slot);
            }
            cnt_inc(cnts, slot);
        } else if (MPOS_TRUTHY) {
            has_mpos = false;
            reset_cols();
        }
    };
    for (;;) {
        while (!pending_close && i < e) {
            const uint32_t fl = r.z & 0xFFu;
            if (!whole && !(fl & MC_RF_CAND)) e = i + 1;
            const bool same_read = started;
            if (!same_read) {
                first_ind = (int)r.y;
                if (fl & MC_RF_BADIDX) sticky_err |= MC_CE_BADNUM;
            }
            if (!same_read) rev = !(fl & MC_RF_EQ);
            else {
                if (fl & MC_RF_BADIDX) sticky_err |= MC_CE_BADNUM;
                rev = !((int)r.y > first_ind);
            }
            cid = (int)r.w;
            pos = (int)r.x;
            const uint32_t bits = rev ? ((r.z >> 16) & 0xFFu) : ((r.z >> 8) & 0xFFu);
            first_m = bits ? (__ffs(bits) - 1) : -1;
            if (MPOS_TRUTHY && pos >= mpos + 1 && same_read) {
                pending_close = true;
                break;
            }
            feed();
            advance();
        }
        const bool pending_handoff = !pending_close && i >= e && !handoff_done && MPOS_TRUTHY;
        if (!pending_close && !pending_handoff) break;
        uint32_t close_idx = i;
        int chrom = cid;
        if (pending_handoff) {
            int64_t j = seg + 1;
            while (j < n_seg && seg_qual[j] < qual_thresh) ++j;
            if (j < n_seg) {
                close_idx = seg_start[j];
                chrom = load_rec(rec + close_idx).contig;
            } else {
                close_idx = 0xFFFFFFFFu;
                chrom = -1;
            }
        }
        emit_window(close_idx, chrom, i);
        if (pending_handoff) {
            handoff_done = true;
            continue;
        }
        if (first_m < 0 || pos > mpos + skip_thresh + 1) {
            reset_cols();
            has_mpos = false;
        } else {
            if (first_m != 0) emit_multi();
            const int last_mpos = mpos;
            mpos = pos + first_m;
            int sp = mpos - last_mpos;
            if (sp > k) sp = k;
            if (sp <= 0) { sticky_err |= MC_CE_SPACING; sp = k; }
            uint32_t nmp = 0u;
            for (int c = 0; c < k; ++c) {
                int slot;
                if (c < sp) { slot = map_get(mp, k - sp + c); cnt_clear(cnts, slot); }
                else slot = map_get(mp, c - sp);
                nmp |= (uint32_t)slot << (4 * c);
            }
            mp = nmp | (mp & ~((k < 8) ? ((1u << (4 * k)) - 1u) : 0xFFFFFFFFu));
        }
        pending_close = false;
        feed();
        advance();
    }
    if (!WRITE) unit_cnt[b] = n_out;
    my_rows += (int)n_out;
#undef MPOS_TRUTHY
    }
    if (!WRITE) {
        __syncthreads();
        int total;
        (void)mc_block_exscan<WIN_THREADS>(my_rows, s_warp, total);
        if (threadIdx.x == 0) blk_tot[blockIdx.x] = (uint32_t)total;
    }
}

__global__ void k_check_cap(const unsigned long long *d_ncalls, unsigned long long cap, unsigned long long *d_flag) {
    if (d_ncalls[0] > cap) *d_flag = 1ull;
}

}

extern "C" int64_t mc_windows_workspace_bytes(int64_t rec_cap) {
    if (rec_cap < 1) rec_cap = 1;
    auto up = [](int64_t bytes) { return ((bytes + 255) / 256) * 256; };
    const int64_t nb = (rec_cap + WIN_RECS - 1) / WIN_RECS;
    return up(rec_cap * 4) + up(rec_cap * 4) + up(2 * nb * 4) + up(rec_cap) + 256 + mc_exscan_ws_bytes(nb) + 512;
}

extern "C" int mc_build_windows(const mc_record *d_rec, const uint64_t *d_n_records, int64_t rec_cap, const uint32_t *d_seg_start,
                                const uint64_t *d_nseg, int64_t seg_cap, const double *d_seg_qual, const mc_refindex *ref,
                                int skip_thresh, double qual_thresh, int two_models, mc_call *d_calls, int64_t call_cap,
                                uint32_t *d_seg_count, uint64_t *d_ncalls, void *d_ws, double *d_spill, int64_t spill_cap,
                                void *stream) {
    MC_REQUIRE(d_rec && d_n_records && d_seg_start && d_nseg && d_seg_qual && ref && d_calls && d_seg_count && d_ncalls && d_ws,
               "null pointer");
    MC_REQUIRE(ref->k >= 1 && ref->k <= MC_MAXK, "k out of range");
    MC_REQUIRE(skip_thresh >= 0, "skip_thresh must be >= 0");
    MC_REQUIRE(spill_cap == 0 || d_spill, "spill arena missing");
    cudaStream_t st = (cudaStream_t)stream;
    MC_CUDA_CHECK(cudaMemsetAsync(d_ncalls, 0, 16, st));
    if (seg_cap <= 0 || rec_cap <= 0) return MC_OK;
    MC_REQUIRE(rec_cap < (1ll << 32), "record count must fit 32 bits");
    if (seg_cap > rec_cap) seg_cap = rec_cap;
    const unsigned long long *dn = reinterpret_cast<const unsigned long long *>(d_n_records);
    const unsigned long long *ds = reinterpret_cast<const unsigned long long *>(d_nseg);
    const int64_t nb = (rec_cap + WIN_RECS - 1) / WIN_RECS;
    auto up = [](int64_t bytes) { return ((bytes + 255) / 256) * 256; };
    uint8_t *w = reinterpret_cast<uint8_t *>(d_ws);
    uint32_t *unit_cnt = reinterpret_cast<uint32_t *>(w);
    int32_t *first_ind = reinterpret_cast<int32_t *>(w + up(rec_cap * 4));
    uint32_t *blk_tot = reinterpret_cast<uint32_t *>(w + 2 * up(rec_cap * 4));
    uint32_t *blk_off = blk_tot + nb;
    uint8_t *tags = w + 2 * up(rec_cap * 4) + up(2 * nb * 4);
    unsigned long long *spill_cursor = reinterpret_cast<unsigned long long *>(tags + up(rec_cap));
    void *scan_ws = reinterpret_cast<uint8_t *>(spill_cursor) + 256;
    MC_CUDA_CHECK(cudaMemsetAsync(spill_cursor, 0, 8, st));
    const Spill spill{d_spill, (unsigned long long)spill_cap, spill_cursor};
    uint32_t *first_idx = d_seg_count;
    k_first_m<<<(unsigned)((seg_cap + 127) / 128), 128, 0, st>>>(d_rec, d_seg_start, seg_cap, ds, first_idx, first_ind);
    MC_LAUNCH_CHECK();
    constexpr size_t rec_bytes = sizeof(uint4) * WIN_RECS, diff_bytes = sizeof(double) * (WIN_RECS + MC_MAXK * WIN_THREADS);
    MC_CUDA_CHECK(cudaFuncSetAttribute(k_windows<false>, cudaFuncAttributeMaxDynamicSharedMemorySize, (int)rec_bytes));
    MC_CUDA_CHECK(cudaFuncSetAttribute(k_windows<true>, cudaFuncAttributeMaxDynamicSharedMemorySize, (int)(rec_bytes + diff_bytes)));
    k_windows<false><<<(unsigned)nb, WIN_THREADS, rec_bytes, st>>>(d_rec, rec_cap, dn, d_seg_start, seg_cap, ds, d_seg_qual, first_idx, first_ind,
                                                          *ref, skip_thresh, qual_thresh, two_models, d_calls,
                                                          (unsigned long long)call_cap, unit_cnt, blk_tot, nullptr, tags, spill);
    MC_LAUNCH_CHECK();
    int rc = mc_exscan_u32(blk_tot, blk_off, nb, nullptr, d_ncalls, scan_ws, st);
    if (rc) return rc;
    k_windows<true><<<(unsigned)nb, WIN_THREADS, rec_bytes + diff_bytes, st>>>(d_rec, rec_cap, dn, d_seg_start, seg_cap, ds, d_seg_qual, first_idx,
                                                                  first_ind, *ref, skip_thresh, qual_thresh, two_models, d_calls,
                                                                  (unsigned long long)call_cap, unit_cnt, nullptr, blk_off, tags, spill);
    MC_LAUNCH_CHECK();
    k_check_cap<<<1, 1, 0, st>>>(reinterpret_cast<unsigned long long *>(d_ncalls), (unsigned long long)call_cap,
                                 reinterpret_cast<unsigned long long *>(d_ncalls) + 1);
    MC_LAUNCH_CHECK();
    return MC_OK;
}
```

### mcaller_b200/engine.py

```python
import ctypes as C

import numpy as np
import torch

from . import _lib
from ._lib import CALL_DTYPE, CARRY_BYTES, MC_C_COUNT, MC_TEXT_PAD, RECORD_DTYPE, check

C_LINES, C_KEPT, C_RECORDS, C_SHORT, C_UNKNOWN, C_NNN, C_BADPOS, C_LONGLINE, C_OVERFLOW = range(9)

S_NSEG, S_MISSING_QUAL, S_NCALLS, S_CALL_OVERFLOW, S_ABORT, S_NREC, S_NROWS = 16, 17, 18, 19, 20, 21, 22
S_STATS = 24
S_WORDS = 32
P_ROW_BASE, P_N_ODD, P_POISON = 0, 1, 2
SPILL_CAP = 1 << 22
ODD_CAP = 1 << 16


def require_cuda():
    if not torch.cuda.is_available():
        raise _lib.McallerCudaError("mcaller_b200 needs a CUDA device (B200, sm_100a); there is no CPU fallback")


class ChunkResult(object):
    __slots__ = ("n_calls", "n_records", "n_segments", "counters", "calls_dev", "missing_quality", "stats", "nbytes")

    def calls(self):
        if self.n_calls == 0:
            return np.zeros(0, dtype=CALL_DTYPE)
        raw = self.calls_dev[: self.n_calls * CALL_DTYPE.itemsize].cpu().numpy()
        return raw.view(CALL_DTYPE)


class Engine(object):
    def __init__(self, refindex, models=None, qual_table=None, skip_thresh=0, qual_thresh=0.0, two_models=False,
                 device="cuda", dense=None, histogram=True):
        require_cuda()
        self.L = _lib.lib()
        self.ref = refindex
        self.models = models
        self.device = torch.device(device)
        if self.device.index is None:
            self.device = torch.device("cuda", torch.cuda.current_device())
        if refindex.device != self.device:
            raise ValueError("reference index lives on %s, engine on %s" % (refindex.device, self.device))
        self.skip_thresh = int(skip_thresh)
        self.qual_thresh = float(qual_thresh)
        self.two_models = 1 if two_models else 0
        self.dense = bool(dense) if dense is not None else False
        self.scan_mode = 1 if self.dense else (2 if self.qual_thresh > 0.0 else 0)
        with torch.cuda.device(self.device):
            if qual_table is None:
                qual_table = np.zeros(16, dtype=_lib.QUAL_DTYPE)
            if hasattr(qual_table, "table") and hasattr(qual_table, "size"):
                self.qual_table_size = int(qual_table.size)
                self.d_qual = qual_table.table
            else:
                self.qual_table_size = len(qual_table)
                self.d_qual = torch.from_numpy(qual_table.view(np.uint8).reshape(-1).copy()).to(self.device)
            self.histogram = histogram
            ns = max(refindex.n_sites, 1)
            self.d_counts = torch.zeros(2 * ns, dtype=torch.int32, device=self.device)
            self.d_depth, self.d_meth = self.d_counts[:ns], self.d_counts[ns:]
            self.d_first = torch.full((ns,), 2 ** 63 - 1, dtype=torch.int64, device=self.device)
            self._bufs = {}
            self.d_small = torch.zeros(S_WORDS, dtype=torch.int64, device=self.device)
            self.d_persist = torch.zeros(8, dtype=torch.int64, device=self.device)
            self.d_carry = torch.zeros(CARRY_BYTES, dtype=torch.uint8, device=self.device)
            self.d_carry_out = torch.zeros(CALL_DTYPE.itemsize, dtype=torch.uint8, device=self.device)
            self.d_odd = torch.zeros(ODD_CAP * CALL_DTYPE.itemsize, dtype=torch.uint8, device=self.device)
            self.d_spill = torch.zeros(SPILL_CAP, dtype=torch.float64, device=self.device)
            self.h_small = np.zeros(S_WORDS, dtype=np.uint64)
            self.rec_per_byte = self.call_per_byte = self.seg_per_byte = 0.0
            self.launches = 0
            self.redone = 0
            self.scan_events = None
            self.reset_stream_state()

    def _buf(self, name, nbytes):
        nbytes = int(max(nbytes, 256))
        t = self._bufs.get(name)
        if t is None or t.numel() < nbytes:
            t = torch.empty(int(nbytes * 1.25) + 256, dtype=torch.uint8, device=self.device)
            self._bufs[name] = t
        return t

    def _sptr(self):
        return C.c_void_p(torch.cuda.current_stream(self.device).cuda_stream)

    def _status_ptr(self, slot):
        return C.c_void_p(self.d_small.data_ptr() + 8 * slot)

    def _persist_ptr(self, slot):
        return C.c_void_p(self.d_persist.data_ptr() + 8 * slot)

    def _read_status(self):
        check(self.L.mc_read_u64(C.c_void_p(self.d_small.data_ptr()), S_WORDS, self.h_small.ctypes.data_as(C.c_void_p), self._sptr()))
        return self.h_small

    @staticmethod
    def padded_capacity(nbytes):
        return ((nbytes + 15) // 16) * 16 + MC_TEXT_PAD + 64

    def upload(self, data):
        n = len(data)
        t = torch.full((self.padded_capacity(n),), 10, dtype=torch.uint8, device=self.device)
        if n:
            t[:n] = torch.from_numpy(np.frombuffer(data, dtype=np.uint8).copy()).to(self.device)
        return t

    def reset_stream_state(self, row_base=0):
        check(self.L.mc_carry_reset(C.c_void_p(self.d_carry.data_ptr()), self._sptr()))
        self.d_persist[:2].zero_()
        if row_base:
            self.d_persist[P_ROW_BASE] = int(row_base)
        self.launches += 1

    def reset_histogram(self, row_base=0):
        self.d_counts.zero_()
        self.d_first.fill_(2 ** 63 - 1)
        self.reset_stream_state(row_base)

    def carry_state(self):
        tail = self.d_carry[CALL_DTYPE.itemsize:CALL_DTYPE.itemsize + 8].cpu().numpy()
        return bool(tail.view(np.uint32)[0]), int(tail.view(np.int32)[1])

    def first_kept_contig_dev(self):
        return self.d_carry[CALL_DTYPE.itemsize + 4:CALL_DTYPE.itemsize + 8].view(torch.int32).to(torch.int64)

    def close_carry(self, closing_contig=-1, next_contigs=None, start=0, fetch=True):
        hist = self.histogram and self.models is not None
        cnt = int(next_contigs.numel()) if next_contigs is not None else 0
        check(self.L.mc_carry_close(C.c_void_p(self.d_carry.data_ptr()), int(closing_contig),
                                    C.c_void_p(next_contigs.data_ptr()) if next_contigs is not None else None, int(start), cnt,
                                    C.c_void_p(self.d_carry_out.data_ptr()),
                                    C.c_void_p(self.d_depth.data_ptr()) if hist else None, C.c_void_p(self.d_meth.data_ptr()) if hist else None,
                                    C.c_void_p(self.d_first.data_ptr()) if hist else None, self.ref.n_sites,
                                    self._persist_ptr(P_ROW_BASE), self._sptr()))
        self.launches += 1
        if not fetch:
            return None
        return self.d_carry_out.cpu().numpy().view(CALL_DTYPE)

    def _default_rec_cap(self, nbytes, n_tiles):
        slack = 256 * min(n_tiles, 8192) + 4096
        return (nbytes // 24 + slack) if self.dense else (nbytes // 1024 + 2 * n_tiles + slack)

    def _caps(self, nbytes, n_tiles):
        slack = 256 * min(n_tiles, 8192) + 4096
        if self.rec_per_byte:
            rec_cap = int(self.rec_per_byte * nbytes * 1.25) + slack
            call_cap = int(self.call_per_byte * nbytes * 1.25) + 1024
            seg_cap = int(self.seg_per_byte * nbytes * 1.5) + 1024
        else:
            rec_cap = self._default_rec_cap(nbytes, n_tiles)
            call_cap = rec_cap // 8 + 1024
            seg_cap = rec_cap
        rec_cap = int(min(max(rec_cap, 1), 2 ** 32 - 2))
        return rec_cap, int(max(call_cap, 1)), int(min(max(seg_cap, 1), rec_cap))

    def run_chunk(self, d_text, nbytes, rec_cap=None, call_cap=None):
        L = self.L
        if d_text.numel() < nbytes + MC_TEXT_PAD:
            raise ValueError("text tensor lacks the MC_TEXT_PAD newline padding")
        res = ChunkResult()
        res.nbytes = nbytes
        n_tiles = int(L.mc_num_tiles(nbytes))
        slack = 256 * min(n_tiles, 8192) + 4096
        if rec_cap is None and call_cap is None:
            rec_cap, call_cap, seg_cap = self._caps(nbytes, n_tiles)
        else:
            d_rec, d_call, d_seg = self._caps(nbytes, n_tiles)
            rec_cap = int(min(max(rec_cap if rec_cap is not None else d_rec, 1), 2 ** 32 - 2))
            call_cap = int(max(call_cap if call_cap is not None else d_call, 1))
            seg_cap = int(min(d_seg, rec_cap))
        attempts = 0
        while True:
            cnt = self._launch_chunk(d_text, nbytes, n_tiles, rec_cap, call_cap, seg_cap)
            reserved, n_rec, n_calls, n_seg = int(cnt[C_RECORDS]), int(cnt[S_NREC]), int(cnt[S_NCALLS]), int(cnt[S_NSEG])
            if nbytes > 0:
                self.rec_per_byte = max(self.rec_per_byte, reserved / nbytes)
                self.call_per_byte = max(self.call_per_byte, n_calls / nbytes)
                self.seg_per_byte = max(self.seg_per_byte, n_seg / nbytes)
            if not cnt[S_ABORT]:
                break
            self.redone += 1
            attempts += 1
            if attempts > 6:
                raise _lib.McallerCudaError("chunk keeps overflowing its buffers (counters: %s)" % list(map(int, cnt[:MC_C_COUNT])))
            if cnt[C_OVERFLOW] or reserved > rec_cap:
                if rec_cap >= 2 ** 32 - 2:
                    raise _lib.McallerCudaError("chunk produces more than 2^32 records; use smaller chunks")
                rec_cap = int(min(max(reserved, rec_cap * 2 if cnt[C_OVERFLOW] and reserved <= rec_cap else 0) + slack, 2 ** 32 - 2))
                call_cap = max(call_cap, rec_cap // 8 + 1024)
            elif n_seg > seg_cap:
                seg_cap = min(n_seg + 1024, rec_cap)
            else:
                call_cap = n_calls + 1024
        if attempts:
            self.d_persist[P_POISON] = 0
        res.counters = {nm: int(cnt[i]) for i, nm in enumerate(_lib.COUNTER_NAMES)}
        res.n_records = n_rec
        res.n_segments = int(cnt[S_NSEG])
        res.missing_quality = int(cnt[S_MISSING_QUAL])
        res.n_calls = int(cnt[S_NROWS])
        res.calls_dev = self._bufs["calls"]
        v = cnt[S_STATS:S_STATS + 7]
        res.stats = dict(calls=int(v[0]), pending=int(v[1]), too_many_skips=int(v[2]), multi=int(v[3]), errors=int(v[4]), methylated=int(v[5]),
                         pending_too_many_skips=int(v[6]))
        return res

    def _launch_chunk(self, d_text, nbytes, n_tiles, rec_cap, call_cap, seg_cap, read_status=True):
        L, st = self.L, self._sptr()
        V = C.c_void_p
        tile_tab = self._buf("tile_tab", 8 * max(n_tiles, 1))
        run_len = max(int(L.mc_scan_run_len(nbytes)), 1)
        n_runs = max((n_tiles + run_len - 1) // run_len, 1)
        run_tab = self._buf("run_tab", 8 * n_runs)
        run_first = self._buf("run_first", 4 * n_runs)
        rec_a = self._buf("rec_a", 32 * rec_cap)
        rec_b = self._buf("rec_b", 32 * rec_cap)
        ws = self._buf("ws", L.mc_workspace_bytes(max(rec_cap, n_tiles)))
        seg_start = self._buf("seg_start", 4 * (rec_cap + 2))
        seg_flags = self._buf("seg_flags", 4 * rec_cap)
        seg_qual = self._buf("seg_qual", 8 * seg_cap)
        seg_count = self._buf("seg_count", 4 * seg_cap)
        calls = self._buf("calls", CALL_DTYPE.itemsize * (call_cap + 1))
        self.d_small.zero_()
        if self.scan_events is not None:
            e0, e1 = torch.cuda.Event(enable_timing=True), torch.cuda.Event(enable_timing=True)
            e0.record()
        check(L.mc_scan(V(d_text.data_ptr()), nbytes, self.ref.ref(), self.scan_mode, V(rec_a.data_ptr()), rec_cap,
                        V(tile_tab.data_ptr()), V(run_tab.data_ptr()), V(self.d_small.data_ptr()), st))
        if self.scan_events is not None:
            e1.record()
            self.scan_events.append((e0, e1))
        check(L.mc_order_records(V(d_text.data_ptr()), nbytes, self.ref.ref(), V(tile_tab.data_ptr()), n_tiles, V(run_tab.data_ptr()), run_len, V(rec_a.data_ptr()), rec_cap,
                                 V(self.d_small.data_ptr()), V(rec_b.data_ptr()), rec_cap, self._status_ptr(S_NREC), V(seg_flags.data_ptr()),
                                 V(run_first.data_ptr()), V(ws.data_ptr()), st))
        check(L.mc_segment_reads(V(d_text.data_ptr()), V(rec_b.data_ptr()), self._status_ptr(S_NREC), rec_cap, V(seg_flags.data_ptr()), V(run_first.data_ptr()),
                                 n_runs if n_tiles else 0, V(seg_start.data_ptr()),
                                 self._status_ptr(S_NSEG), V(ws.data_ptr()), st))
        check(L.mc_segment_quality(V(d_text.data_ptr()), V(rec_b.data_ptr()), V(seg_start.data_ptr()), self._status_ptr(S_NSEG), seg_cap,
                                   V(self.d_qual.data_ptr()), self.qual_table_size, V(seg_qual.data_ptr()), self._status_ptr(S_MISSING_QUAL), st))
        rows1 = V(calls.data_ptr() + CALL_DTYPE.itemsize)
        check(L.mc_build_windows(V(rec_b.data_ptr()), self._status_ptr(S_NREC), rec_cap, V(seg_start.data_ptr()), self._status_ptr(S_NSEG),
                                 seg_cap, V(seg_qual.data_ptr()), self.ref.ref(), self.skip_thresh, self.qual_thresh, self.two_models,
                                 rows1, call_cap, V(seg_count.data_ptr()), self._status_ptr(S_NCALLS), V(ws.data_ptr()),
                                 V(self.d_spill.data_ptr()), SPILL_CAP, st))
        check(L.mc_chunk_guard(V(self.d_small.data_ptr()), rec_cap, self._status_ptr(S_NREC), rec_cap, self._status_ptr(S_NSEG), seg_cap,
                               self._status_ptr(S_NCALLS), call_cap, self._status_ptr(S_ABORT), self._persist_ptr(P_POISON), st))
        check(L.mc_carry_rows(V(calls.data_ptr()), self._status_ptr(S_NCALLS), V(rec_b.data_ptr()), self._status_ptr(S_NREC),
                              V(seg_start.data_ptr()), self._status_ptr(S_NSEG), V(seg_qual.data_ptr()), self.qual_thresh,
                              V(self.d_carry.data_ptr()), self._status_ptr(S_NROWS), self._status_ptr(S_ABORT), st))
        self.launches += 1 + 5 + 5 + 1 + 7 + 2
        if self.models is not None:
            cls_ws = self._buf("cls_ws", L.mc_classify_workspace_bytes(call_cap + 1))
            check(L.mc_classify(V(calls.data_ptr()), self._status_ptr(S_NROWS), call_cap + 1, self.models.array, V(cls_ws.data_ptr()), st))
            self.launches += 2
            if self.histogram:
                check(L.mc_hist_accumulate(V(calls.data_ptr()), self._status_ptr(S_NROWS), call_cap + 1, V(self.d_depth.data_ptr()),
                                           V(self.d_meth.data_ptr()), V(self.d_first.data_ptr()), self.ref.n_sites, self._persist_ptr(P_ROW_BASE),
                                           V(self.d_odd.data_ptr()), ODD_CAP, self._persist_ptr(P_N_ODD), self._status_ptr(S_ABORT), st))
                self.launches += 2
        check(L.mc_count_calls(V(calls.data_ptr()), self._status_ptr(S_NROWS), call_cap + 1, self._status_ptr(S_STATS), st))
        self.launches += 1
        if not read_status:
            return None
        return self._read_status().copy()

    def launch_chunk(self, d_text, nbytes):
        if not self.rec_per_byte:
            raise _lib.McallerCudaError("launch_chunk needs a preceding run_chunk (capacities are learned from it)")
        n_tiles = int(self.L.mc_num_tiles(nbytes))
        rec_cap, call_cap, seg_cap = self._caps(nbytes, n_tiles)
        self._launch_chunk(d_text, nbytes, n_tiles, rec_cap, call_cap, seg_cap, read_status=False)

    def overflowed(self, clear=True):
        v = int(self.d_persist[P_POISON].item())
        if clear and v:
            self.d_persist[P_POISON] = 0
        return bool(v)

    def count_rows(self, res):
        return dict(res.stats)

    def records(self, n_rec):
        return self._bufs["rec_b"][: n_rec * 32].cpu().numpy().view(RECORD_DTYPE)

    def histogram_host(self):
        return (self.d_depth.cpu().numpy().view(np.uint32), self.d_meth.cpu().numpy().view(np.uint32),
                self.d_first.cpu().numpy().view(np.uint64))

    def bed_select(self, depth_thresh, mod_thresh, control=False):
        ns = max(self.ref.n_sites, 1)
        if getattr(self, "d_bed_flags", None) is None:
            self.d_bed_flags = torch.zeros(ns, dtype=torch.uint8, device=self.device)
            self.d_bed_count = torch.zeros(1, dtype=torch.int64, device=self.device)
        check(self.L.mc_bed_select(C.c_void_p(self.d_depth.data_ptr()), C.c_void_p(self.d_meth.data_ptr()), self.ref.n_sites, int(depth_thresh),
                                   float(mod_thresh), 1 if control else 0, C.c_void_p(self.d_bed_flags.data_ptr()),
                                   C.c_void_p(self.d_bed_count.data_ptr()), self._sptr()))
        self.launches += 1
        return self.d_bed_flags, self.d_bed_count

    def odd_rows(self):
        n = int(self.d_persist[P_N_ODD].item())
        if n > ODD_CAP:
            raise _lib.McallerCudaError("more than %d rows close on another contig than their window's" % ODD_CAP)
        return self.d_odd[: n * CALL_DTYPE.itemsize].cpu().numpy().view(CALL_DTYPE)
```

Baseline: 49.15 million.

## Fuse MLP classification into single-pass staged window builder

Replaces the two-pass count-then-write window kernel with a single pass that writes rows into a per-block staging buffer and then places them with a small copy kernel. When both models are one-hidden-layer MLPs, classification runs inside the window kernel using weights staged in the record shared memory, and only the chunk-edge rows are reclassified by a tiny edge kernel. The aim is to avoid recomputing windows, the separate classify pass and its index compaction, at the cost of extra staging memory, an adaptive stage size learned from past chunks, and more shared-memory pressure.

Result: slower. 48.29 million, median of 6 (-1.8%).

```diff
diff --git a/include/mcaller_b200.h b/include/mcaller_b200.h
--- a/include/mcaller_b200.h
+++ b/include/mcaller_b200.h
@@ -163,10 +163,14 @@
                        int64_t seg_cap, const mc_qual_entry *d_table, int64_t table_size, double *d_seg_qual, uint64_t *d_err,
                        void *stream);
 
-int mc_build_windows(const mc_record *d_rec, const uint64_t *d_n_records, int64_t rec_cap, const uint32_t *d_seg_start,
-                     const uint64_t *d_nseg, int64_t seg_cap, const double *d_seg_qual, const mc_refindex *ref, int skip_thresh,
-                     double qual_thresh, int two_models, mc_call *d_calls, int64_t call_cap, uint32_t *d_seg_count,
-                     uint64_t *d_ncalls, void *d_ws, double *d_spill, int64_t spill_cap, void *stream);
+int64_t mc_windows_stage_bytes(int64_t rec_cap, int64_t stage_rows);
+int mc_windows_classifies(const mc_model *models);
+int mc_build_windows_staged(const mc_record *d_rec, const uint64_t *d_n_records, int64_t rec_cap, const uint32_t *d_seg_start,
+                            const uint64_t *d_nseg, int64_t seg_cap, const double *d_seg_qual, const mc_refindex *ref,
+                            int skip_thresh, double qual_thresh, int two_models, mc_call *d_calls, int64_t call_cap,
+                            uint32_t *d_seg_count, uint64_t *d_ncalls, void *d_ws, double *d_spill, int64_t spill_cap,
+                            mc_call *d_stage, int64_t stage_rows, uint64_t *d_blk_rows, const mc_model *models ,
+                            void *stream);
 
 typedef struct mc_carry {
     mc_call row;
@@ -187,6 +191,7 @@
 
 int64_t mc_classify_workspace_bytes(int64_t row_cap);
 int mc_classify(mc_call *d_calls, const uint64_t *d_nrows, int64_t row_cap, const mc_model *models, void *d_ws, void *stream);
+int mc_classify_edges(mc_call *d_calls, const uint64_t *d_nrows, int64_t row_cap, const mc_model *models, void *stream);
 
 int mc_hist_accumulate(const mc_call *d_calls, const uint64_t *d_nrows, int64_t row_cap, uint32_t *d_depth, uint32_t *d_meth,
                        uint64_t *d_first, int64_t n_sites, uint64_t *d_row_base, mc_call *d_odd, int64_t odd_cap, uint64_t *d_n_odd,
diff --git a/mcaller_b200/_lib.py b/mcaller_b200/_lib.py
--- a/mcaller_b200/_lib.py
+++ b/mcaller_b200/_lib.py
@@ -97,9 +97,11 @@
                                    C.c_void_p, C.c_void_p]),
     "mc_segment_quality": (C.c_int, [C.c_void_p, C.c_void_p, C.c_void_p, C.c_void_p, C.c_int64, C.c_void_p, C.c_int64, C.c_void_p,
                                      C.c_void_p, C.c_void_p]),
-    "mc_build_windows": (C.c_int, [C.c_void_p, C.c_void_p, C.c_int64, C.c_void_p, C.c_void_p, C.c_int64, C.c_void_p, C.POINTER(RefIndex),
+    "mc_windows_stage_bytes": (C.c_int64, [C.c_int64, C.c_int64]),
+    "mc_windows_classifies": (C.c_int, [C.POINTER(Model)]),
+    "mc_build_windows_staged": (C.c_int, [C.c_void_p, C.c_void_p, C.c_int64, C.c_void_p, C.c_void_p, C.c_int64, C.c_void_p, C.POINTER(RefIndex),
                                    C.c_int, C.c_double, C.c_int, C.c_void_p, C.c_int64, C.c_void_p, C.c_void_p, C.c_void_p, C.c_void_p,
-                                   C.c_int64, C.c_void_p]),
+                                   C.c_int64, C.c_void_p, C.c_int64, C.c_void_p, C.POINTER(Model), C.c_void_p]),
     "mc_carry_reset": (C.c_int, [C.c_void_p, C.c_void_p]),
     "mc_carry_rows": (C.c_int, [C.c_void_p, C.c_void_p, C.c_void_p, C.c_void_p, C.c_void_p, C.c_void_p, C.c_void_p, C.c_double, C.c_void_p,
                                 C.c_void_p, C.c_void_p, C.c_void_p]),
@@ -109,6 +111,7 @@
                                  C.c_int64, C.c_void_p, C.c_void_p]),
     "mc_classify_workspace_bytes": (C.c_int64, [C.c_int64]),
     "mc_classify": (C.c_int, [C.c_void_p, C.c_void_p, C.c_int64, C.POINTER(Model), C.c_void_p, C.c_void_p]),
+    "mc_classify_edges": (C.c_int, [C.c_void_p, C.c_void_p, C.c_int64, C.POINTER(Model), C.c_void_p]),
     "mc_hist_accumulate": (C.c_int, [C.c_void_p, C.c_void_p, C.c_int64, C.c_void_p, C.c_void_p, C.c_void_p, C.c_int64, C.c_void_p,
                                      C.c_void_p, C.c_int64, C.c_void_p, C.c_void_p, C.c_void_p]),
     "mc_count_calls": (C.c_int, [C.c_void_p, C.c_void_p, C.c_int64, C.c_void_p, C.c_void_p]),
diff --git a/mcaller_b200/csrc/classify.cu b/mcaller_b200/csrc/classify.cu
--- a/mcaller_b200/csrc/classify.cu
+++ b/mcaller_b200/csrc/classify.cu
@@ -4,15 +4,6 @@
 
 constexpr int MAX_WIDTH = 512;
 constexpr int WARPS = 8;
-
-__device__ __forceinline__ double activate(double v, int act) {
-    switch (act) {
-        case MC_ACT_TANH: return mc_tanh(v);
-        case MC_ACT_LOGISTIC: return mc_expit(v);
-        case MC_ACT_RELU: return v > 0.0 ? v : 0.0;
-        default: return v;
-    }
-}
 
 template <bool STAGED>
 __global__ void __launch_bounds__(WARPS * 32)
@@ -78,7 +69,7 @@
                             const int o = o0 + lane + 32 * j;
                             if (o < no) {
                                 const double z = acc[j] + ld(bi + o);
-                                y[o] = last ? z : activate(z, m.hidden_act);
+                                y[o] = last ? z : mc_activate(z, m.hidden_act);
                             }
                         }
                     }
@@ -88,7 +79,7 @@
                         for (int k = lane; k < ni; k += 32) acc = fma(x[k], ld(w + (size_t)k * no + o), acc);
                         for (int d = 16; d > 0; d >>= 1) acc += __shfl_xor_sync(0xffffffffu, acc, d);
                         acc += ld(bi + o);
-                        if (lane == 0) y[o] = last ? acc : activate(acc, m.hidden_act);
+                        if (lane == 0) y[o] = last ? acc : mc_activate(acc, m.hidden_act);
                     }
                 }
                 __syncwarp();
@@ -108,8 +99,6 @@
         ks_cur = ks_next;
     }
 }
-
-constexpr int MLP_MAX_IN = MC_MAXK + 1;
 
 __global__ void __launch_bounds__(256) k_call_index(const mc_call *__restrict__ calls, int64_t n_cap, const unsigned long long *__restrict__ d_n,
                                                    uint32_t *__restrict__ idx, unsigned long long *__restrict__ d_nidx) {
@@ -137,63 +126,56 @@
     extern __shared__ __align__(16) double s_mlp[];
     const int64_t n = (int64_t)*d_nidx;
     if ((int64_t)blockIdx.x * WARPS * 8 >= n) return;
-    for (int j = threadIdx.x; j < nw0; j += WARPS * 32) s_mlp[j] = __ldg(m0.d_weights + j);
-    for (int j = threadIdx.x; j < nb0; j += WARPS * 32) s_mlp[nw0 + j] = __ldg(m0.d_biases + j);
-    for (int j = threadIdx.x; j < nw1; j += WARPS * 32) s_mlp[nw0 + nb0 + j] = __ldg(m1.d_weights + j);
-    for (int j = threadIdx.x; j < nb1; j += WARPS * 32) s_mlp[nw0 + nb0 + nw1 + j] = __ldg(m1.d_biases + j);
+    mc_stage_mlp1(s_mlp, m0, m1, nw0, nb0, nw1, nb1);
     __syncthreads();
     const int warp = threadIdx.x >> 5, lane = threadIdx.x & 31, g = lane & 3, grp = lane >> 2;
     const int64_t stride = (int64_t)gridDim.x * WARPS * 8;
     for (int64_t base = ((int64_t)blockIdx.x * WARPS + warp) * 8; base < n; base += stride) {
         int64_t i = base + grp;
         int ks = -1;
-        double x[MLP_MAX_IN];
-#pragma unroll
-        for (int k = 0; k < MLP_MAX_IN; ++k) x[k] = 0.0;
+        double x[MC_MLP1_MAX_IN];
+#pragma unroll
+        for (int k = 0; k < MC_MLP1_MAX_IN; ++k) x[k] = 0.0;
         if (i < n) {
             i = (int64_t)__ldg(idx + i);
             const mc_call &c = calls[i];
             ks = (int)c.model_sel;
 #pragma unroll
-            for (int k = 0; k < MLP_MAX_IN; ++k) x[k] = c.feat[k];
-        }
-        const bool second = ks > 0;
-        const mc_model &m = second ? m1 : m0;
-        const int ni = m.sizes[0], H = m.sizes[1], act = m.hidden_act;
-        const double *w0 = (second && !alias) ? s_mlp + nw0 + nb0 : s_mlp;
-        const double *b0 = (second && !alias) ? s_mlp + nw0 + nb0 + nw1 : s_mlp + nw0;
-        const double *w1 = w0 + (size_t)ni * H, *b1 = b0 + H;
-        double out = 0.0;
-        if (ks >= 0) {
-            for (int o0 = g; o0 < H; o0 += 16) {
-                double z[4];
-#pragma unroll
-                for (int j = 0; j < 4; ++j) z[j] = 0.0;
-#pragma unroll
-                for (int k = 0; k < MLP_MAX_IN; ++k) {
-                    if (k < ni) {
-#pragma unroll
-                        for (int j = 0; j < 4; ++j) {
-                            const int o = o0 + 4 * j;
-                            if (o < H) z[j] = fma(x[k], w0[(size_t)k * H + o], z[j]);
-                        }
-                    }
-                }
-#pragma unroll
-                for (int j = 0; j < 4; ++j) {
-                    const int o = o0 + 4 * j;
-                    if (o < H) out = fma(act == MC_ACT_TANH ? mc_tanh(z[j] + b0[o]) : activate(z[j] + b0[o], act), w1[o], out);
-                }
-            }
-        }
-        out += __shfl_xor_sync(0xffffffffu, out, 1);
-        out += __shfl_xor_sync(0xffffffffu, out, 2);
+            for (int k = 0; k < MC_MLP1_MAX_IN; ++k) x[k] = c.feat[k];
+        }
+        const double p = mc_mlp1_prob(x, ks, m0, m1, s_mlp, nw0, nb0, nw1, alias);
         if (ks >= 0 && g == 0) {
-            const double p = mc_expit(out + b1[0]);
             mc_call &c = calls[i];
             c.prob = p;
             c.label = (uint8_t)(p >= 0.5);
         }
+    }
+}
+
+__global__ void __launch_bounds__(32)
+k_mlp1_edges(mc_call *__restrict__ calls, int64_t n_cap, const unsigned long long *__restrict__ d_n, mc_model m0, mc_model m1, int nw0,
+             int nb0, int nw1, int nb1, int alias) {
+    extern __shared__ __align__(16) double s_mlp[];
+    const int64_t n = mc_dev_count(d_n, n_cap);
+    if (n <= 0) return;
+    mc_stage_mlp1(s_mlp, m0, m1, nw0, nb0, nw1, nb1);
+    __syncthreads();
+    const int grp = threadIdx.x >> 2;
+    const int64_t i = grp == 0 ? 0 : (grp == 1 ? n - 1 : -1);
+    int ks = -1;
+    double x[MC_MLP1_MAX_IN];
+#pragma unroll
+    for (int k = 0; k < MC_MLP1_MAX_IN; ++k) x[k] = 0.0;
+    if (i >= 0 && i < n && !(grp == 1 && i == 0) && calls[i].kind == MC_CALL) {
+        const mc_call &c = calls[i];
+        ks = (int)c.model_sel;
+#pragma unroll
+        for (int k = 0; k < MC_MLP1_MAX_IN; ++k) x[k] = c.feat[k];
+    }
+    const double p = mc_mlp1_prob(x, ks, m0, m1, s_mlp, nw0, nb0, nw1, alias);
+    if (ks >= 0 && (threadIdx.x & 3) == 0) {
+        calls[i].prob = p;
+        calls[i].label = (uint8_t)(p >= 0.5);
     }
 }
 
@@ -530,6 +512,36 @@
     return MC_OK;
 }
 
+bool mc_mlp1_shape(const mc_model *models, size_t smem_limit, int &nw0, int &nb0, int &nw1, int &nb1, int &alias) {
+    const mc_model &m0 = models[0], &m1 = models[1];
+    if (m0.kind != MC_MLP || m1.kind != MC_MLP || m0.n_in < 1 || m0.n_in > MC_MLP1_MAX_IN || m1.n_in != m0.n_in) return false;
+    for (const mc_model *m : {&m0, &m1}) {
+        if (m->n_layers != 2 || m->sizes[0] != m->n_in || m->sizes[2] != 1) return false;
+        for (int l = 0; l <= 2; ++l)
+            if (m->sizes[l] < 1 || m->sizes[l] > MAX_WIDTH) return false;
+    }
+    alias = m1.d_weights == m0.d_weights ? 1 : 0;
+    nw0 = m0.sizes[0] * m0.sizes[1] + m0.sizes[1];
+    nb0 = m0.sizes[1] + 1;
+    nw1 = alias ? 0 : m1.sizes[0] * m1.sizes[1] + m1.sizes[1];
+    nb1 = alias ? 0 : m1.sizes[1] + 1;
+    return sizeof(double) * (size_t)(nw0 + nb0 + nw1 + nb1) <= smem_limit;
+}
+
+extern "C" int mc_classify_edges(mc_call *d_calls, const uint64_t *d_nrows, int64_t row_cap, const mc_model *models, void *stream) {
+    MC_REQUIRE(d_calls && d_nrows && models, "null pointer");
+    int nw0, nb0, nw1, nb1, alias;
+    MC_REQUIRE(mc_mlp1_shape(models, MC_WIN_MLP_BYTES, nw0, nb0, nw1, nb1, alias),
+               "models are not one-hidden-layer MLPs that mc_build_windows_staged classifies");
+    if (row_cap <= 0) return MC_OK;
+    const size_t bytes = sizeof(double) * (size_t)(nw0 + nb0 + nw1 + nb1);
+    MC_CUDA_CHECK(cudaFuncSetAttribute(k_mlp1_edges, cudaFuncAttributeMaxDynamicSharedMemorySize, (int)bytes));
+    k_mlp1_edges<<<1, 32, bytes, (cudaStream_t)stream>>>(d_calls, row_cap, reinterpret_cast<const unsigned long long *>(d_nrows), models[0],
+                                                        models[1], nw0, nb0, nw1, nb1, alias);
+    MC_LAUNCH_CHECK();
+    return MC_OK;
+}
+
 extern "C" int64_t mc_classify_workspace_bytes(int64_t row_cap) { return 256 + 4 * (row_cap < 1 ? 1 : row_cap); }
 
 extern "C" int mc_classify(mc_call *d_calls, const uint64_t *d_nrows, int64_t n_calls , const mc_model *models,
@@ -571,11 +583,9 @@
             const size_t staged_bytes = act_bytes + sizeof(double) * (size_t)(nw0 + nb0 + nw1 + nb1);
             int64_t blocks = (n_calls + WARPS - 1) / WARPS;
             if (blocks > (int64_t)sms * 8) blocks = (int64_t)sms * 8;
-            auto one_hidden = [](const mc_model &m) {
-                return m.kind == MC_MLP && m.n_layers == 2 && m.sizes[0] <= MLP_MAX_IN && m.sizes[2] == 1;
-            };
             const size_t weight_bytes = sizeof(double) * (size_t)(nw0 + nb0 + nw1 + nb1);
-            if (one_hidden(m0) && (alias || one_hidden(m1)) && weight_bytes <= 100 * 1024) {
+            int s_nw0, s_nb0, s_nw1, s_nb1, s_alias;
+            if (mc_mlp1_shape(models, 100 * 1024, s_nw0, s_nb0, s_nw1, s_nb1, s_alias)) {
                 int64_t b2 = (n_calls + WARPS * 8 - 1) / (WARPS * 8);
                 if (b2 > (int64_t)sms * 8) b2 = (int64_t)sms * 8;
                 unsigned long long *d_nidx = reinterpret_cast<unsigned long long *>(d_ws);
diff --git a/mcaller_b200/csrc/common.cuh b/mcaller_b200/csrc/common.cuh
--- a/mcaller_b200/csrc/common.cuh
+++ b/mcaller_b200/csrc/common.cuh
@@ -182,3 +182,60 @@
     q = fma(fma(-d, q, u), rc, q);
     return copysign(q, x);
 }
+
+__device__ __forceinline__ double mc_activate(double v, int act) {
+    switch (act) {
+        case MC_ACT_TANH: return mc_tanh(v);
+        case MC_ACT_LOGISTIC: return mc_expit(v);
+        case MC_ACT_RELU: return v > 0.0 ? v : 0.0;
+        default: return v;
+    }
+}
+
+constexpr int MC_MLP1_MAX_IN = MC_MAXK + 1;
+__device__ __forceinline__ double mc_mlp1_prob(const double (&x)[MC_MLP1_MAX_IN], int ks, const mc_model &m0, const mc_model &m1,
+                                               const double *s_mlp, int nw0, int nb0, int nw1, int alias) {
+    const int g = threadIdx.x & 3;
+    const bool second = ks > 0;
+    const mc_model &m = second ? m1 : m0;
+    const int ni = m.sizes[0], H = m.sizes[1], act = m.hidden_act;
+    const double *w0 = (second && !alias) ? s_mlp + nw0 + nb0 : s_mlp;
+    const double *b0 = (second && !alias) ? s_mlp + nw0 + nb0 + nw1 : s_mlp + nw0;
+    const double *w1 = w0 + (size_t)ni * H, *b1 = b0 + H;
+    double out = 0.0;
+    if (ks >= 0) {
+        for (int o0 = g; o0 < H; o0 += 16) {
+            double z[4];
+#pragma unroll
+            for (int j = 0; j < 4; ++j) z[j] = 0.0;
+#pragma unroll
+            for (int k = 0; k < MC_MLP1_MAX_IN; ++k) {
+                if (k < ni) {
+#pragma unroll
+                    for (int j = 0; j < 4; ++j) {
+                        const int o = o0 + 4 * j;
+                        if (o < H) z[j] = fma(x[k], w0[(size_t)k * H + o], z[j]);
+                    }
+                }
+            }
+#pragma unroll
+            for (int j = 0; j < 4; ++j) {
+                const int o = o0 + 4 * j;
+                if (o < H) out = fma(act == MC_ACT_TANH ? mc_tanh(z[j] + b0[o]) : mc_activate(z[j] + b0[o], act), w1[o], out);
+            }
+        }
+    }
+    out += __shfl_xor_sync(0xffffffffu, out, 1);
+    out += __shfl_xor_sync(0xffffffffu, out, 2);
+    return ks >= 0 ? mc_expit(out + b1[0]) : 0.0;
+}
+
+__device__ __forceinline__ void mc_stage_mlp1(double *s_mlp, const mc_model &m0, const mc_model &m1, int nw0, int nb0, int nw1, int nb1) {
+    for (int j = threadIdx.x; j < nw0; j += blockDim.x) s_mlp[j] = __ldg(m0.d_weights + j);
+    for (int j = threadIdx.x; j < nb0; j += blockDim.x) s_mlp[nw0 + j] = __ldg(m0.d_biases + j);
+    for (int j = threadIdx.x; j < nw1; j += blockDim.x) s_mlp[nw0 + nb0 + j] = __ldg(m1.d_weights + j);
+    for (int j = threadIdx.x; j < nb1; j += blockDim.x) s_mlp[nw0 + nb0 + nw1 + j] = __ldg(m1.d_biases + j);
+}
+
+constexpr size_t MC_WIN_MLP_BYTES = 32 * 1024;
+bool mc_mlp1_shape(const mc_model *models, size_t smem_limit, int &nw0, int &nb0, int &nw1, int &nb1, int &alias);
diff --git a/mcaller_b200/csrc/windows.cu b/mcaller_b200/csrc/windows.cu
--- a/mcaller_b200/csrc/windows.cu
+++ b/mcaller_b200/csrc/windows.cu
@@ -15,6 +15,8 @@
 constexpr int WIN_UNITS = WIN_RECS / 2 + 2;
 static_assert(WIN_RECS < 65536, "unit / read counts of a block are packed in 16 bits");
 constexpr uint32_t TAG_NONE = 0xFu;
+constexpr size_t WIN_DYN_BYTES = sizeof(uint4) * WIN_RECS + sizeof(double) * (WIN_RECS + MC_MAXK * WIN_THREADS);
+static_assert(MC_WIN_MLP_BYTES <= WIN_DYN_BYTES, "the classifier's weights are staged where the records were");
 
 __device__ __forceinline__ uint4 stage_word(const mc_record *p) {
     const uint4 a = __ldg(reinterpret_cast<const uint4 *>(p)), b = __ldg(reinterpret_cast<const uint4 *>(p) + 1);
@@ -141,35 +143,75 @@
     return mc_pairwise_sum([a](int64_t q) { return a[q]; }, 0, n);
 }
 
-template <bool WRITE>
+struct WinMlp {
+    mc_model m0, m1;
+    int nw0, nb0, nw1, nb1, alias, on;
+};
+
+
+__device__ __forceinline__ void classify_rows(mc_call *rows, int n, const double *s_mlp, const WinMlp &P) {
+    const int lane = threadIdx.x & 31, grp = lane >> 2;
+    for (int b0 = (threadIdx.x >> 5) * 32; b0 < n; b0 += WIN_THREADS) {
+        const int r = b0 + lane;
+        bool want = false;
+        if (r < n) want = rows[r].kind == MC_CALL && rows[r].close_rec != 0xFFFFFFFFu;
+        for (uint32_t m = __ballot_sync(0xffffffffu, want); m;) {
+            uint32_t mm = m;
+            for (int t = 0; t < grp && mm; ++t) mm &= mm - 1u;
+            const int my = mm ? b0 + __ffs(mm) - 1 : -1;
+            for (int t = 0; t < 8 && m; ++t) m &= m - 1u;
+            int ks = -1;
+            double x[MC_MLP1_MAX_IN];
+#pragma unroll
+            for (int k = 0; k < MC_MLP1_MAX_IN; ++k) x[k] = 0.0;
+            if (my >= 0) {
+                const mc_call &c = rows[my];
+                ks = (int)c.model_sel;
+#pragma unroll
+                for (int k = 0; k < MC_MLP1_MAX_IN; ++k) x[k] = c.feat[k];
+            }
+            const double p = mc_mlp1_prob(x, ks, P.m0, P.m1, s_mlp, P.nw0, P.nb0, P.nw1, P.alias);
+            if (my >= 0 && (lane & 3) == 0) {
+                rows[my].prob = p;
+                rows[my].label = (uint8_t)(p >= 0.5);
+            }
+        }
+    }
+}
+
 __global__ void __launch_bounds__(WIN_THREADS, MC_WIN_BLOCKS)
 k_windows(const mc_record *__restrict__ rec, int64_t rec_cap, const unsigned long long *__restrict__ d_n_records,
           const uint32_t *__restrict__ seg_start, int64_t seg_cap, const unsigned long long *__restrict__ d_nseg,
           const double *__restrict__ seg_qual, const uint32_t *__restrict__ first_idx, const int32_t *__restrict__ first_ind_arr,
           mc_refindex R, int skip_thresh, double qual_thresh, int two_models, mc_call *__restrict__ calls,
-          unsigned long long call_cap, uint32_t *__restrict__ unit_cnt ,
-          uint32_t *__restrict__ blk_tot, const uint32_t *__restrict__ blk_off, uint8_t *__restrict__ g_tag , Spill spill) {
+          unsigned long long call_cap, mc_call *__restrict__ stage , uint32_t stage_cap,
+          uint32_t *__restrict__ blk_tot ,
+          unsigned long long *__restrict__ d_ncalls, unsigned long long *__restrict__ d_blk_rows, uint8_t *__restrict__ g_tag ,
+          Spill spill, WinMlp mlp) {
     __shared__ uint32_t s_unit[WIN_UNITS];
     __shared__ uint32_t s_off[WIN_UNITS];
     __shared__ uint16_t s_seg[WIN_UNITS];
     __shared__ int s_warp[WIN_THREADS / 32 + 1];
     __shared__ int64_t s_seg0;
+    __shared__ uint32_t s_nrows;
     extern __shared__ __align__(16) uint4 s_dyn[];
     uint4 *s_rec = s_dyn;
     double *s_diff = reinterpret_cast<double *>(s_dyn + WIN_RECS);
     double *s_seq = s_diff + WIN_RECS + threadIdx.x;
     const int k = R.k;
+    if (threadIdx.x == 0) s_nrows = 0u;
+    __syncthreads();
+    const uint32_t blk = blockIdx.x;
+    mc_call *const my_stage = stage + (size_t)blk * stage_cap;
     const int64_t n_records = mc_dev_count(d_n_records, rec_cap), n_seg = mc_dev_count(d_nseg, seg_cap);
-    const int64_t base = (int64_t)blockIdx.x * WIN_RECS;
-    if (base >= n_records || n_seg <= 0) {
-        if (!WRITE && threadIdx.x == 0) blk_tot[blockIdx.x] = 0u;
-        return;
-    }
+    const int64_t base = (int64_t)blk * WIN_RECS;
+    int nu = 0;
+    if (base < n_records && n_seg > 0) {
     for (int j = threadIdx.x; j < WIN_RECS; j += WIN_THREADS) {
         const int64_t i = base + j;
         if (i < n_records) {
             s_rec[j] = stage_word(rec + i);
-            if (WRITE) s_diff[j] = stage_diff(rec + i);
+            s_diff[j] = stage_diff(rec + i);
         } else {
             s_rec[j] = make_uint4(0u, 0u, TAG_NONE << 24, 0u);
         }
@@ -189,18 +231,13 @@
     };
     auto rec_diff = [&](uint32_t i) -> double {
         const int64_t j = (int64_t)i - base;
-        return (WRITE && j >= 0 && j < WIN_RECS) ? s_diff[j] : stage_diff(rec + i);
+        return (j >= 0 && j < WIN_RECS) ? s_diff[j] : stage_diff(rec + i);
     };
     auto tag_set = [&](uint32_t i, uint32_t t) {
         const int64_t j = (int64_t)i - base;
         if (j >= 0 && j < WIN_RECS) s_rec[j].z = (s_rec[j].z & 0x00FFFFFFu) | (t << 24);
         else g_tag[i] = (uint8_t)t;
     };
-    auto tag_get = [&](uint32_t i) -> uint32_t {
-        const int64_t j = (int64_t)i - base;
-        return (j >= 0 && j < WIN_RECS) ? (s_rec[j].z >> 24) : (uint32_t)g_tag[i];
-    };
-    int nu;
     {
         const int j0 = threadIdx.x * WIN_ITEMS;
         const int64_t i0 = base + j0;
@@ -243,27 +280,6 @@
         if (nu > WIN_UNITS) nu = WIN_UNITS;
         __syncthreads();
     }
-    if (WRITE) {
-        constexpr int UPT = (WIN_UNITS + WIN_THREADS - 1) / WIN_THREADS;
-        uint32_t v[UPT];
-        int sum = 0;
-#pragma unroll
-        for (int j = 0; j < UPT; ++j) {
-            const int u = threadIdx.x * UPT + j;
-            v[j] = u < nu ? unit_cnt[s_unit[u]] : 0u;
-            sum += (int)v[j];
-        }
-        int total;
-        uint32_t run = blk_off[blockIdx.x] + (uint32_t)mc_block_exscan<WIN_THREADS>(sum, s_warp, total);
-#pragma unroll
-        for (int j = 0; j < UPT; ++j) {
-            const int u = threadIdx.x * UPT + j;
-            if (u < WIN_UNITS) s_off[u] = run;
-            run += v[j];
-        }
-        __syncthreads();
-    }
-    int my_rows = 0;
     for (int un = threadIdx.x; un < nu; un += WIN_THREADS) {
     const uint32_t b = s_unit[un];
     const int64_t seg = s_seg0 + s_seg[un];
@@ -272,11 +288,10 @@
     uint32_t n_out = 0;
     const double myq = seg_qual[seg];
     if (myq < qual_thresh || (whole && b != seg_b)) {
-        if (!WRITE) unit_cnt[b] = 0u;
+        s_off[un] = 0u;
         continue;
     }
     uint32_t e = e_read;
-    uint32_t out_pos = WRITE ? s_off[un] : 0u;
     const uint32_t fidx = __ldg(first_idx + seg);
 
     Counts cnts{0ull, 0ull};
@@ -300,12 +315,15 @@
         return __ddiv_rn(res, (double)n);
     };
 
+    auto row_slot = [&]() -> mc_call * {
+        const uint32_t slot = atomicAdd(&s_nrows, 1u);
+        return slot < stage_cap ? my_stage + slot : nullptr;
+    };
     auto emit_window = [&](uint32_t close_idx, int chrom_cid, uint32_t upto) {
         int n_empty = 0;
         for (int c = 0; c < k; ++c) n_empty += (cnt_get(cnts, map_get(mp, c)) == 0);
-        if (WRITE) {
-            if (out_pos < call_cap) {
-                mc_call &o = calls[out_pos];
+        if (mc_call *const op = row_slot()) {
+                mc_call &o = *op;
                 const mc_record nr = load_rec(rec + name_rec);
                 o.read_off = mc_rec_line(nr) + nr.name_off;
                 o.read_len = nr.name_len;
@@ -319,8 +337,8 @@
                 o.label = 0;
                 o.pad0 = 0;
                 o.seg = (uint32_t)seg;
-                o.pad1 = 0;
-                o.pad2 = 0;
+                o.pad1 = (uint32_t)un;
+                o.pad2 = n_out;
                 uint32_t err = sticky_err;
                 uint32_t empty_mask = 0u;
                 const int64_t g = __ldg(R.d_base + last_cid) + mpos;
@@ -361,15 +379,12 @@
                 }
                 o.empty_mask = (uint8_t)empty_mask;
                 o.err = (uint8_t)err;
-            }
-            ++out_pos;
         }
         ++n_out;
     };
     auto emit_multi = [&]() {
-        if (WRITE) {
-            if (out_pos < call_cap) {
-                mc_call &o = calls[out_pos];
+        if (mc_call *const op = row_slot()) {
+                mc_call &o = *op;
                 const mc_record nr = load_rec(rec + name_rec);
                 o.read_off = mc_rec_line(nr) + nr.name_off;
                 o.read_len = nr.name_len;
@@ -384,17 +399,15 @@
                 o.rev = (uint8_t)last_rev;
                 o.n_empty = 0; o.empty_mask = 0; o.model_sel = 0; o.label = 0; o.err = 0; o.pad0 = 0;
                 o.seg = (uint32_t)seg;
-                o.pad1 = 0;
-                o.pad2 = 0;
-            }
-            ++out_pos;
+                o.pad1 = (uint32_t)un;
+                o.pad2 = n_out;
         }
         ++n_out;
     };
     auto reset_cols = [&]() { cnts.lo = 0ull; cnts.hi = 0ull; };
 
     auto tag_init = [&](uint32_t q) {
-        if (WRITE && (int64_t)q - base >= WIN_RECS) g_tag[q] = (uint8_t)TAG_NONE;
+        if ((int64_t)q - base >= WIN_RECS) g_tag[q] = (uint8_t)TAG_NONE;
     };
     uint32_t i = b;
     uint4 r = (b < e) ? rec_word(b) : make_uint4(0u, 0u, 0u, 0u);
@@ -415,7 +428,7 @@
             name_rec = i;
             if (r.z & MC_RF_BADNUM) sticky_err |= MC_CE_BADNUM;
             const int slot = map_get(mp, first_m);
-            if (WRITE) {
+            {
                 const double v = rec_diff(i);
                 double *q = s_seq + slot * WIN_THREADS;
                 *q = __dadd_rn(cnt_get(cnts, slot) == 0 ? 0.0 : *q, v);
@@ -495,20 +508,69 @@
         feed();
         advance();
     }
-    if (!WRITE) unit_cnt[b] = n_out;
-    my_rows += (int)n_out;
+    s_off[un] = n_out;
 #undef MPOS_TRUTHY
     }
-    if (!WRITE) {
+    }
+    __syncthreads();
+    constexpr int UPT = (WIN_UNITS + WIN_THREADS - 1) / WIN_THREADS;
+    uint32_t v[UPT];
+    int sum = 0;
+#pragma unroll
+    for (int j = 0; j < UPT; ++j) {
+        const int u = threadIdx.x * UPT + j;
+        v[j] = u < nu ? s_off[u] : 0u;
+        sum += (int)v[j];
+    }
+    int total;
+    uint32_t run = (uint32_t)mc_block_exscan<WIN_THREADS>(sum, s_warp, total);
+#pragma unroll
+    for (int j = 0; j < UPT; ++j) {
+        const int u = threadIdx.x * UPT + j;
+        if (u < WIN_UNITS) s_off[u] = run;
+        run += v[j];
+    }
+    __syncthreads();
+    const int n_staged = total < (int)stage_cap ? total : (int)stage_cap;
+    for (int r = threadIdx.x; r < n_staged; r += WIN_THREADS) {
+        uint2 *t = reinterpret_cast<uint2 *>(&my_stage[r].pad1);
+        const uint2 v = *t;
+        *t = make_uint2(s_off[v.x] + v.y, 0u);
+    }
+    if (threadIdx.x == 0) {
+        blk_tot[blk] = (uint32_t)total;
+        if (total > (int)stage_cap) d_ncalls[1] = 1ull;
+        if ((unsigned long long)total > *reinterpret_cast<volatile unsigned long long *>(d_blk_rows))
+            atomicMax(d_blk_rows, (unsigned long long)total);
+    }
+    if (mlp.on && n_staged > 0) {
+        double *s_mlp = reinterpret_cast<double *>(s_dyn);
+        mc_stage_mlp1(s_mlp, mlp.m0, mlp.m1, mlp.nw0, mlp.nb0, mlp.nw1, mlp.nb1);
         __syncthreads();
-        int total;
-        (void)mc_block_exscan<WIN_THREADS>(my_rows, s_warp, total);
-        if (threadIdx.x == 0) blk_tot[blockIdx.x] = (uint32_t)total;
-    }
-}
-
-__global__ void k_check_cap(const unsigned long long *d_ncalls, unsigned long long cap, unsigned long long *d_flag) {
-    if (d_ncalls[0] > cap) *d_flag = 1ull;
+        classify_rows(my_stage, n_staged, s_mlp, mlp);
+    }
+}
+
+__global__ void __launch_bounds__(128)
+k_place_rows(const mc_call *__restrict__ stage, uint32_t stage_cap, const uint32_t *__restrict__ blk_tot, const uint32_t *__restrict__ blk_off,
+             mc_call *__restrict__ calls, unsigned long long call_cap, unsigned long long *__restrict__ d_ncalls) {
+    if (blockIdx.x == 0 && threadIdx.x == 0 && d_ncalls[0] > call_cap) d_ncalls[1] = 1ull;
+    const uint32_t n = blk_tot[blockIdx.x] < stage_cap ? blk_tot[blockIdx.x] : stage_cap;
+    const unsigned long long base = blk_off[blockIdx.x];
+    const mc_call *src = stage + (size_t)blockIdx.x * stage_cap;
+    for (uint32_t r = threadIdx.x; r < n; r += blockDim.x) {
+        const uint4 *s4 = reinterpret_cast<const uint4 *>(src + r);
+        uint4 q[8];
+#pragma unroll
+        for (int j = 0; j < 8; ++j) q[j] = s4[j];
+        const unsigned long long dst = base + q[7].z;
+        q[7].z = 0u;
+        if (dst < call_cap) {
+            uint4 *d = reinterpret_cast<uint4 *>(calls + dst);
+#pragma unroll
+            for (int j = 0; j < 8; ++j) d[j] = q[j];
+        }
+    }
 }
 
 }
@@ -517,19 +579,39 @@
     if (rec_cap < 1) rec_cap = 1;
     auto up = [](int64_t bytes) { return ((bytes + 255) / 256) * 256; };
     const int64_t nb = (rec_cap + WIN_RECS - 1) / WIN_RECS;
-    return up(rec_cap * 4) + up(rec_cap * 4) + up(2 * nb * 4) + up(rec_cap) + 256 + mc_exscan_ws_bytes(nb) + 512;
-}
-
-extern "C" int mc_build_windows(const mc_record *d_rec, const uint64_t *d_n_records, int64_t rec_cap, const uint32_t *d_seg_start,
-                                const uint64_t *d_nseg, int64_t seg_cap, const double *d_seg_qual, const mc_refindex *ref,
-                                int skip_thresh, double qual_thresh, int two_models, mc_call *d_calls, int64_t call_cap,
-                                uint32_t *d_seg_count, uint64_t *d_ncalls, void *d_ws, double *d_spill, int64_t spill_cap,
-                                void *stream) {
-    MC_REQUIRE(d_rec && d_n_records && d_seg_start && d_nseg && d_seg_qual && ref && d_calls && d_seg_count && d_ncalls && d_ws,
-               "null pointer");
+    return up(rec_cap * 4) + up(rec_cap) + up(2 * nb * 4) + 256 + mc_exscan_ws_bytes(nb) + 512;
+}
+
+extern "C" int64_t mc_windows_stage_bytes(int64_t rec_cap, int64_t stage_rows) {
+    if (rec_cap < 1) rec_cap = 1;
+    if (stage_rows < 1) stage_rows = 1;
+    return (rec_cap + WIN_RECS - 1) / WIN_RECS * stage_rows * (int64_t)sizeof(mc_call);
+}
+
+extern "C" int mc_windows_classifies(const mc_model *models) {
+    int nw0, nb0, nw1, nb1, alias;
+    return models && mc_mlp1_shape(models, MC_WIN_MLP_BYTES, nw0, nb0, nw1, nb1, alias) ? 1 : 0;
+}
+
+extern "C" int mc_build_windows_staged(const mc_record *d_rec, const uint64_t *d_n_records, int64_t rec_cap, const uint32_t *d_seg_start,
+                                       const uint64_t *d_nseg, int64_t seg_cap, const double *d_seg_qual, const mc_refindex *ref,
+                                       int skip_thresh, double qual_thresh, int two_models, mc_call *d_calls, int64_t call_cap,
+                                       uint32_t *d_seg_count, uint64_t *d_ncalls, void *d_ws, double *d_spill, int64_t spill_cap,
+                                       mc_call *d_stage, int64_t stage_rows, uint64_t *d_blk_rows, const mc_model *models, void *stream) {
+    MC_REQUIRE(d_rec && d_n_records && d_seg_start && d_nseg && d_seg_qual && ref && d_calls && d_seg_count && d_ncalls && d_ws &&
+               d_stage && d_blk_rows, "null pointer");
     MC_REQUIRE(ref->k >= 1 && ref->k <= MC_MAXK, "k out of range");
     MC_REQUIRE(skip_thresh >= 0, "skip_thresh must be >= 0");
     MC_REQUIRE(spill_cap == 0 || d_spill, "spill arena missing");
+    MC_REQUIRE(stage_rows >= 1 && stage_rows < (1ll << 31), "stage_rows out of range");
+    WinMlp mlp{};
+    if (models) {
+        MC_REQUIRE(mc_mlp1_shape(models, MC_WIN_MLP_BYTES, mlp.nw0, mlp.nb0, mlp.nw1, mlp.nb1, mlp.alias),
+                   "models are not one-hidden-layer MLPs the window builder classifies (see mc_windows_classifies)");
+        mlp.m0 = models[0];
+        mlp.m1 = models[1];
+        mlp.on = 1;
+    }
     cudaStream_t st = (cudaStream_t)stream;
     MC_CUDA_CHECK(cudaMemsetAsync(d_ncalls, 0, 16, st));
     if (seg_cap <= 0 || rec_cap <= 0) return MC_OK;
@@ -540,33 +622,27 @@
     const int64_t nb = (rec_cap + WIN_RECS - 1) / WIN_RECS;
     auto up = [](int64_t bytes) { return ((bytes + 255) / 256) * 256; };
     uint8_t *w = reinterpret_cast<uint8_t *>(d_ws);
-    uint32_t *unit_cnt = reinterpret_cast<uint32_t *>(w);
-    int32_t *first_ind = reinterpret_cast<int32_t *>(w + up(rec_cap * 4));
-    uint32_t *blk_tot = reinterpret_cast<uint32_t *>(w + 2 * up(rec_cap * 4));
+    int32_t *first_ind = reinterpret_cast<int32_t *>(w);
+    uint8_t *tags = w + up(rec_cap * 4);
+    uint32_t *blk_tot = reinterpret_cast<uint32_t *>(tags + up(rec_cap));
     uint32_t *blk_off = blk_tot + nb;
-    uint8_t *tags = w + 2 * up(rec_cap * 4) + up(2 * nb * 4);
-    unsigned long long *spill_cursor = reinterpret_cast<unsigned long long *>(tags + up(rec_cap));
+    unsigned long long *spill_cursor = reinterpret_cast<unsigned long long *>(tags + up(rec_cap) + up(2 * nb * 4));
     void *scan_ws = reinterpret_cast<uint8_t *>(spill_cursor) + 256;
     MC_CUDA_CHECK(cudaMemsetAsync(spill_cursor, 0, 8, st));
     const Spill spill{d_spill, (unsigned long long)spill_cap, spill_cursor};
     uint32_t *first_idx = d_seg_count;
     k_first_m<<<(unsigned)((seg_cap + 127) / 128), 128, 0, st>>>(d_rec, d_seg_start, seg_cap, ds, first_idx, first_ind);
     MC_LAUNCH_CHECK();
-    constexpr size_t rec_bytes = sizeof(uint4) * WIN_RECS, diff_bytes = sizeof(double) * (WIN_RECS + MC_MAXK * WIN_THREADS);
-    MC_CUDA_CHECK(cudaFuncSetAttribute(k_windows<false>, cudaFuncAttributeMaxDynamicSharedMemorySize, (int)rec_bytes));
-    MC_CUDA_CHECK(cudaFuncSetAttribute(k_windows<true>, cudaFuncAttributeMaxDynamicSharedMemorySize, (int)(rec_bytes + diff_bytes)));
-    k_windows<false><<<(unsigned)nb, WIN_THREADS, rec_bytes, st>>>(d_rec, rec_cap, dn, d_seg_start, seg_cap, ds, d_seg_qual, first_idx, first_ind,
-                                                          *ref, skip_thresh, qual_thresh, two_models, d_calls,
-                                                          (unsigned long long)call_cap, unit_cnt, blk_tot, nullptr, tags, spill);
+    MC_CUDA_CHECK(cudaFuncSetAttribute(k_windows, cudaFuncAttributeMaxDynamicSharedMemorySize, (int)WIN_DYN_BYTES));
+    k_windows<<<(unsigned)nb, WIN_THREADS, WIN_DYN_BYTES, st>>>(
+        d_rec, rec_cap, dn, d_seg_start, seg_cap, ds, d_seg_qual, first_idx, first_ind, *ref, skip_thresh, qual_thresh, two_models, d_calls,
+        (unsigned long long)call_cap, d_stage, (uint32_t)stage_rows, blk_tot, reinterpret_cast<unsigned long long *>(d_ncalls),
+        reinterpret_cast<unsigned long long *>(d_blk_rows), tags, spill, mlp);
     MC_LAUNCH_CHECK();
     int rc = mc_exscan_u32(blk_tot, blk_off, nb, nullptr, d_ncalls, scan_ws, st);
     if (rc) return rc;
-    k_windows<true><<<(unsigned)nb, WIN_THREADS, rec_bytes + diff_bytes, st>>>(d_rec, rec_cap, dn, d_seg_start, seg_cap, ds, d_seg_qual, first_idx,
-                                                                  first_ind, *ref, skip_thresh, qual_thresh, two_models, d_calls,
-                                                                  (unsigned long long)call_cap, unit_cnt, nullptr, blk_off, tags, spill);
-    MC_LAUNCH_CHECK();
-    k_check_cap<<<1, 1, 0, st>>>(reinterpret_cast<unsigned long long *>(d_ncalls), (unsigned long long)call_cap,
-                                 reinterpret_cast<unsigned long long *>(d_ncalls) + 1);
+    k_place_rows<<<(unsigned)nb, 128, 0, st>>>(d_stage, (uint32_t)stage_rows, blk_tot, blk_off, d_calls, (unsigned long long)call_cap,
+                                               reinterpret_cast<unsigned long long *>(d_ncalls));
     MC_LAUNCH_CHECK();
     return MC_OK;
 }
diff --git a/mcaller_b200/engine.py b/mcaller_b200/engine.py
--- a/mcaller_b200/engine.py
+++ b/mcaller_b200/engine.py
@@ -8,12 +8,13 @@
 
 C_LINES, C_KEPT, C_RECORDS, C_SHORT, C_UNKNOWN, C_NNN, C_BADPOS, C_LONGLINE, C_OVERFLOW = range(9)
 
-S_NSEG, S_MISSING_QUAL, S_NCALLS, S_CALL_OVERFLOW, S_ABORT, S_NREC, S_NROWS = 16, 17, 18, 19, 20, 21, 22
+S_NSEG, S_MISSING_QUAL, S_NCALLS, S_CALL_OVERFLOW, S_ABORT, S_NREC, S_NROWS, S_BLK_ROWS = 16, 17, 18, 19, 20, 21, 22, 23
 S_STATS = 24
 S_WORDS = 32
 P_ROW_BASE, P_N_ODD, P_POISON = 0, 1, 2
 SPILL_CAP = 1 << 22
 ODD_CAP = 1 << 16
+STAGE_ROWS = 384
 
 
 def require_cuda():
@@ -71,6 +72,8 @@
             self.d_spill = torch.zeros(SPILL_CAP, dtype=torch.float64, device=self.device)
             self.h_small = np.zeros(S_WORDS, dtype=np.uint64)
             self.rec_per_byte = self.call_per_byte = self.seg_per_byte = 0.0
+            self.blk_rows = 0
+            self.fused_models = models is not None and bool(self.L.mc_windows_classifies(models.array))
             self.launches = 0
             self.redone = 0
             self.scan_events = None
@@ -144,6 +147,9 @@
     def _default_rec_cap(self, nbytes, n_tiles):
         slack = 256 * min(n_tiles, 8192) + 4096
         return (nbytes // 24 + slack) if self.dense else (nbytes // 1024 + 2 * n_tiles + slack)
+
+    def _stage_rows(self):
+        return int(self.blk_rows * 1.25) + 64 if self.blk_rows else STAGE_ROWS
 
     def _caps(self, nbytes, n_tiles):
         slack = 256 * min(n_tiles, 8192) + 4096
@@ -177,6 +183,9 @@
         while True:
             cnt = self._launch_chunk(d_text, nbytes, n_tiles, rec_cap, call_cap, seg_cap)
             reserved, n_rec, n_calls, n_seg = int(cnt[C_RECORDS]), int(cnt[S_NREC]), int(cnt[S_NCALLS]), int(cnt[S_NSEG])
+            stage_rows = self._stage_rows()
+            blk_rows = int(cnt[S_BLK_ROWS])
+            self.blk_rows = max(self.blk_rows, blk_rows)
             if nbytes > 0:
                 self.rec_per_byte = max(self.rec_per_byte, reserved / nbytes)
                 self.call_per_byte = max(self.call_per_byte, n_calls / nbytes)
@@ -194,6 +203,8 @@
                 call_cap = max(call_cap, rec_cap // 8 + 1024)
             elif n_seg > seg_cap:
                 seg_cap = min(n_seg + 1024, rec_cap)
+            elif blk_rows > stage_rows:
+                pass
             else:
                 call_cap = n_calls + 1024
         if attempts:
@@ -225,6 +236,8 @@
         seg_qual = self._buf("seg_qual", 8 * seg_cap)
         seg_count = self._buf("seg_count", 4 * seg_cap)
         calls = self._buf("calls", CALL_DTYPE.itemsize * (call_cap + 1))
+        stage_rows = self._stage_rows()
+        stage = self._buf("stage", L.mc_windows_stage_bytes(rec_cap, stage_rows))
         self.d_small.zero_()
         if self.scan_events is not None:
             e0, e1 = torch.cuda.Event(enable_timing=True), torch.cuda.Event(enable_timing=True)
@@ -243,25 +256,29 @@
         check(L.mc_segment_quality(V(d_text.data_ptr()), V(rec_b.data_ptr()), V(seg_start.data_ptr()), self._status_ptr(S_NSEG), seg_cap,
                                    V(self.d_qual.data_ptr()), self.qual_table_size, V(seg_qual.data_ptr()), self._status_ptr(S_MISSING_QUAL), st))
         rows1 = V(calls.data_ptr() + CALL_DTYPE.itemsize)
-        check(L.mc_build_windows(V(rec_b.data_ptr()), self._status_ptr(S_NREC), rec_cap, V(seg_start.data_ptr()), self._status_ptr(S_NSEG),
+        check(L.mc_build_windows_staged(V(rec_b.data_ptr()), self._status_ptr(S_NREC), rec_cap, V(seg_start.data_ptr()), self._status_ptr(S_NSEG),
                                  seg_cap, V(seg_qual.data_ptr()), self.ref.ref(), self.skip_thresh, self.qual_thresh, self.two_models,
                                  rows1, call_cap, V(seg_count.data_ptr()), self._status_ptr(S_NCALLS), V(ws.data_ptr()),
-                                 V(self.d_spill.data_ptr()), SPILL_CAP, st))
+                                 V(self.d_spill.data_ptr()), SPILL_CAP, V(stage.data_ptr()), stage_rows, self._status_ptr(S_BLK_ROWS),
+                                 self.models.array if self.fused_models else None, st))
         check(L.mc_chunk_guard(V(self.d_small.data_ptr()), rec_cap, self._status_ptr(S_NREC), rec_cap, self._status_ptr(S_NSEG), seg_cap,
                                self._status_ptr(S_NCALLS), call_cap, self._status_ptr(S_ABORT), self._persist_ptr(P_POISON), st))
         check(L.mc_carry_rows(V(calls.data_ptr()), self._status_ptr(S_NCALLS), V(rec_b.data_ptr()), self._status_ptr(S_NREC),
                               V(seg_start.data_ptr()), self._status_ptr(S_NSEG), V(seg_qual.data_ptr()), self.qual_thresh,
                               V(self.d_carry.data_ptr()), self._status_ptr(S_NROWS), self._status_ptr(S_ABORT), st))
-        self.launches += 1 + 5 + 5 + 1 + 7 + 2
-        if self.models is not None:
+        self.launches += 1 + 5 + 5 + 1 + 6 + 2
+        if self.fused_models:
+            check(L.mc_classify_edges(V(calls.data_ptr()), self._status_ptr(S_NROWS), call_cap + 1, self.models.array, st))
+            self.launches += 1
+        elif self.models is not None:
             cls_ws = self._buf("cls_ws", L.mc_classify_workspace_bytes(call_cap + 1))
             check(L.mc_classify(V(calls.data_ptr()), self._status_ptr(S_NROWS), call_cap + 1, self.models.array, V(cls_ws.data_ptr()), st))
             self.launches += 2
-            if self.histogram:
-                check(L.mc_hist_accumulate(V(calls.data_ptr()), self._status_ptr(S_NROWS), call_cap + 1, V(self.d_depth.data_ptr()),
-                                           V(self.d_meth.data_ptr()), V(self.d_first.data_ptr()), self.ref.n_sites, self._persist_ptr(P_ROW_BASE),
-                                           V(self.d_odd.data_ptr()), ODD_CAP, self._persist_ptr(P_N_ODD), self._status_ptr(S_ABORT), st))
-                self.launches += 2
+        if self.models is not None and self.histogram:
+            check(L.mc_hist_accumulate(V(calls.data_ptr()), self._status_ptr(S_NROWS), call_cap + 1, V(self.d_depth.data_ptr()),
+                                       V(self.d_meth.data_ptr()), V(self.d_first.data_ptr()), self.ref.n_sites, self._persist_ptr(P_ROW_BASE),
+                                       V(self.d_odd.data_ptr()), ODD_CAP, self._persist_ptr(P_N_ODD), self._status_ptr(S_ABORT), st))
+            self.launches += 2
         check(L.mc_count_calls(V(calls.data_ptr()), self._status_ptr(S_NROWS), call_cap + 1, self._status_ptr(S_STATS), st))
         self.launches += 1
         if not read_status:
```
